# Pranav-Jain/Neural-Monte-Carlo-Fluid-Simulation

Hardware: AMD Instinct MI355X
Metric: WoS walk-steps/sec + pressure-projection wall-time per step, 2D karman 64k pts (higher is better)
Workload: dtype f32

## Files before the change

### include/wos.h

```cpp
#ifndef WOS_H
#define WOS_H

#include <stdint.h>

#ifdef __cplusplus
extern "C" {
#endif

#define WOS_ABI_VERSION 10

enum {
    WOS_OK = 0,
    WOS_E_INVALID = -1,
    WOS_E_IO = -2,
    WOS_E_DEVICE = -3,
    WOS_E_CAPACITY = -4,
    WOS_E_NOMEM = -5
};

#define WOS_PTRS_DEVICE 0x1u
#define WOS_ASYNC       0x2u

typedef struct wos_mesh {
    int32_t dim;
    int32_t n_vertices;
    int32_t n_prims;
    float *vertices;
    int32_t *prims;
} wos_mesh;

int wos_load_obj(const char *path, int32_t dim, int32_t flip_orientation,
                 int32_t normalize, wos_mesh *out);
void wos_mesh_free(wos_mesh *mesh);

typedef struct wos_scene_desc {
    int32_t dim;
    const float *vertices;
    const int32_t *prims;
    int32_t n_vertices, n_prims;
    const float *dvertices;
    const int32_t *dprims;
    int32_t n_dvertices, n_dprims;
    float dirichlet_value;
    float absorption;
    int32_t is_watertight;
    int32_t is_double_sided;
    const float *source;
    int32_t source_dims[3];
    int32_t source_on_device;
    const float *dirichlet_image;
    int32_t dirichlet_image_dims[2];
    float dirichlet_image_box[4];
    int32_t dirichlet_image_on_device;
    const float *neumann_image;
    int32_t neumann_image_dims[2];
    float neumann_image_box[4];
    int32_t neumann_image_on_device;
} wos_scene_desc;

typedef struct wos_scene wos_scene;

int wos_scene_create(const wos_scene_desc *desc, int32_t device, wos_scene **out);
int wos_scene_destroy(wos_scene *scene);

int wos_scene_set_source(wos_scene *scene, const float *source, const int32_t *dims,
                         int32_t on_device, void *stream);

#define WOS_MAX_CHANNELS 4
int wos_scene_set_source_channels(wos_scene *scene, const float *source, int32_t n_channels,
                                  const int32_t *dims, const float *dirichlet_values,
                                  int32_t on_device, void *stream);
int32_t wos_scene_channels(const wos_scene *scene);

int wos_release_caches(int32_t device);

int64_t wos_set_max_batch_tasks(int64_t max_tasks);

typedef struct wos_scene_info {
    int32_t dim, n_prims, n_silhouettes, n_dprims, device;
    float bbox_min[3], bbox_max[3];
} wos_scene_info;
int wos_scene_get_info(const wos_scene *scene, wos_scene_info *info);

enum { WOS_QUERY_NEUMANN = 0, WOS_QUERY_DIRICHLET = 1 };
int wos_scene_query(wos_scene *scene, int32_t which, float boundary_distance_mask,
                    const float *pts, int64_t n,
                    float *dist, float *signed_dist, float *closest , int32_t *state,
                    void *stream, uint32_t flags);

typedef struct wos_solver_params {
    int32_t n_walks;
    int32_t max_walk_length;
    int32_t steps_before_tikhonov;
    int32_t steps_before_maximal_spheres;
    float epsilon_shell;
    float min_star_radius;
    float silhouette_precision;
    float russian_roulette_threshold;
    float boundary_distance_mask;
    int32_t disable_gradient_control_variates;
    int32_t disable_gradient_antithetic_variates;
    int32_t use_cosine_sampling;
    int32_t ignore_dirichlet;
    int32_t ignore_neumann;
    int32_t ignore_source;
    uint64_t seed;
    int32_t robust_float;
    uint32_t schedule;
} wos_solver_params;

#define WOS_SCHED_GEOM_GLOBAL   0x1u
#define WOS_SCHED_FULL_NEUMANN  0x2u
#define WOS_SCHED_NO_STAR_GRID  0x4u
#define WOS_SCHED_NO_DIR_GRID   0x8u
#define WOS_SCHED_NO_TAIL_SPREAD 0x10u
#define WOS_SCHED_NO_GRID_SPREAD 0x20u

void wos_default_params(wos_solver_params *p);

typedef struct wos_stats {
    uint64_t walk_steps;
    uint64_t wasted_steps;
    uint64_t walks_recorded;
    uint64_t walks_escaped;
    uint64_t walks_max_length;
    uint64_t walks_rr;
    uint64_t walks_dirichlet;
    uint64_t points_estimated;
    uint64_t rejection_iters;
    double kernel_ms;
    double first_ball_ms;
    double walk_ms;
    double fold_ms;
    uint64_t walk_launches;
    int32_t first_ball_blocks_per_cu;
    int32_t walk_blocks_per_cu;
    int32_t walk_lds_bytes;
    int32_t star_grid;
    int32_t geom_global;
    int32_t dir_grid;
    uint64_t ticket;
} wos_stats;

int wos_solve(wos_scene *scene, const wos_solver_params *params,
              const float *pts, int64_t n, int64_t index_base, int64_t index_stride,
              float *p, float *grad, int32_t *n_est, int32_t *steps,
              wos_stats *stats, void *stream, uint32_t flags);

int wos_solve_var(wos_scene *scene, const wos_solver_params *params,
                  const float *pts, int64_t n, int64_t index_base, int64_t index_stride,
                  float *p, float *grad, float *p_var, float *grad_var, int32_t *n_est, int32_t *steps,
                  wos_stats *stats, void *stream, uint32_t flags);

int wos_solve_channels(wos_scene *scene, const wos_solver_params *params,
                       const float *pts, int64_t n, int64_t index_base, int64_t index_stride,
                       int32_t n_channels, float *p, float *grad, float *p_var, float *grad_var,
                       int32_t *n_est, int32_t *steps, wos_stats *stats, void *stream, uint32_t flags);

typedef struct wos_bvc_params {
    int32_t n_walks_solution;
// ... 102 lines not shown
```

### neural-monte-carlo-fluid-simulation_amd/csrc/wos_capi.hip

```cpp
#include <hip/hip_runtime.h>

#include <algorithm>
#include <cmath>
#include <list>
#include <cstdlib>
#include <cstring>
#include <memory>
#include <condition_variable>
#include <atomic>
#include <mutex>
#include <string>
#include <vector>

#include "../../include/wos.h"
#include "wos_bvc.h"
#include "wos_detmath.h"
#include "wos_host_scene.h"
#include "wos_launch.h"
#include "wos_siren.h"

namespace {

thread_local std::string g_err;

int fail(int code, const std::string& msg) {
  g_err = msg;
  return code;
}

#define HIP_TRY(expr)                                                                         \
  do {                                                                                        \
    hipError_t _e = (expr);                                                                   \
    if (_e != hipSuccess) return fail(WOS_E_DEVICE, std::string(#expr ": ") + hipGetErrorString(_e)); \
  } while (0)

template <typename T>
hipError_t upload(T** dst, const std::vector<T>& src) {
  *dst = nullptr;
  if (src.empty()) return hipSuccess;
  hipError_t e = hipMalloc((void**)dst, src.size() * sizeof(T));
  if (e != hipSuccess) { *dst = nullptr; return e; }
  e = hipMemcpy(*dst, src.data(), src.size() * sizeof(T), hipMemcpyHostToDevice);
  if (e != hipSuccess) {
    hipFree(*dst);
    *dst = nullptr;
  }
  return e;
}

struct StatSlot {
  uint64_t ticket = 0;
  unsigned long long* h_cnt = nullptr;
  hipEvent_t ev0 = nullptr, ev1 = nullptr, done = nullptr;
  std::vector<hipEvent_t> bev;
  int64_t n_batches = 0;
  int32_t bpc_fb = 0, bpc_walk = 0, walk_lds = 0, star_grid = 0, geom_global = 0, dir_grid = 0;
};
constexpr int kStatSlots = 16;

struct TaskWs {
  float* tasks = nullptr;
  int64_t task_cap = 0;
  int32_t* pstate = nullptr;
  int64_t pstate_cap = 0;
  unsigned long long* counters = nullptr;
  hipStream_t stream = nullptr;
  hipEvent_t done = nullptr;
};
constexpr int kSideWs = 2;

struct DevCtx {
  std::mutex mu;
  bool ready = false;
  int num_cus = 0;
  float* d_pts = nullptr;
  float* d_p = nullptr;
  float* d_g = nullptr;
  int32_t* d_nest = nullptr;
  int32_t* d_steps = nullptr;
  size_t ws_points = 0;
  float* d_pvar = nullptr;
  float* d_gvar = nullptr;
  size_t ws_var_points = 0;
  uint64_t* d_jump = nullptr;
  int n_jump = 0;
  float* d_tasks = nullptr;
  int64_t task_cap = 0;
  int32_t* d_pstate = nullptr;
  int64_t pstate_cap = 0;
  unsigned long long* d_counters = nullptr;
  StatSlot slot[kStatSlots];
  uint64_t next_ticket = 1;
  hipEvent_t done = nullptr;
  hipStream_t last_stream = nullptr;
  bool inflight = false;
  float* d_rejtab = nullptr;
  int stat_waiters = 0;
  std::condition_variable no_waiters;
  TaskWs side[kSideWs];
  hipStream_t bvc_dir = nullptr;
  hipEvent_t bvc_dir_done = nullptr;
};

constexpr int kMaxDevices = 64;
DevCtx g_ctx[kMaxDevices];

void ctx_free(DevCtx& c) {
  hipFree(c.d_pts); hipFree(c.d_p); hipFree(c.d_g); hipFree(c.d_nest); hipFree(c.d_steps);
  hipFree(c.d_pvar); hipFree(c.d_gvar);
  c.d_pvar = c.d_gvar = nullptr;
  c.ws_var_points = 0;
  hipFree(c.d_jump); hipFree(c.d_tasks); hipFree(c.d_pstate); hipFree(c.d_counters); hipFree(c.d_rejtab);
  c.d_rejtab = nullptr;
  for (StatSlot& q : c.slot) {
    if (q.ev0) hipEventDestroy(q.ev0);
    if (q.ev1) hipEventDestroy(q.ev1);
    if (q.done) hipEventDestroy(q.done);
    for (hipEvent_t e : q.bev) hipEventDestroy(e);
    if (q.h_cnt) hipHostFree(q.h_cnt);
    q = StatSlot{};
  }
  if (c.done) hipEventDestroy(c.done);
  if (c.bvc_dir_done) hipEventDestroy(c.bvc_dir_done);
  if (c.bvc_dir) hipStreamDestroy(c.bvc_dir);
  c.bvc_dir_done = nullptr;
  c.bvc_dir = nullptr;
  for (TaskWs& w : c.side) {
    hipFree(w.tasks); hipFree(w.pstate); hipFree(w.counters);
    if (w.done) hipEventDestroy(w.done);
    if (w.stream) hipStreamDestroy(w.stream);
    w = TaskWs{};
  }
  c.d_pts = c.d_p = c.d_g = nullptr;
  c.d_nest = c.d_steps = nullptr;
  c.ws_points = 0;
  c.d_jump = nullptr; c.n_jump = 0;
  c.d_tasks = nullptr; c.task_cap = 0;
  c.d_pstate = nullptr; c.pstate_cap = 0;
  c.d_counters = nullptr;
  c.done = nullptr;
  c.last_stream = nullptr;
  c.inflight = false;
  c.ready = false;
}

const std::vector<float>& rejection_tables() {
  static std::once_flag once;
  static std::vector<float> t(2 * wos::kRejTabBins);
  std::call_once(once, [] {
    wos::rejection_bound_table(2, t.data());
    wos::rejection_bound_table(3, t.data() + wos::kRejTabBins);
  });
  return t;
}

int ctx_ready(DevCtx& c, int device) {
  if (c.ready) return WOS_OK;
  {
    const std::vector<float>& t = rejection_tables();
    HIP_TRY(hipMalloc((void**)&c.d_rejtab, t.size() * sizeof(float)));
    HIP_TRY(hipMemcpy(c.d_rejtab, t.data(), t.size() * sizeof(float), hipMemcpyHostToDevice));
  }
  HIP_TRY(hipDeviceGetAttribute(&c.num_cus, hipDeviceAttributeMultiprocessorCount, device));
  HIP_TRY(hipMalloc((void**)&c.d_counters, wos::kMainCounterSlots * sizeof(unsigned long long)));
  for (StatSlot& q : c.slot) {
    HIP_TRY(hipHostMalloc((void**)&q.h_cnt, wos::kNumCounters * sizeof(unsigned long long)));
    HIP_TRY(hipEventCreate(&q.ev0));
    HIP_TRY(hipEventCreate(&q.ev1));
    HIP_TRY(hipEventCreateWithFlags(&q.done, hipEventDisableTiming));
  }
  HIP_TRY(hipEventCreateWithFlags(&c.done, hipEventDisableTiming));
  c.ready = true;
  return WOS_OK;
}

hipError_t ctx_order(DevCtx& c, hipStream_t st) {
  if (c.inflight && c.last_stream != st && c.done) return hipStreamWaitEvent(st, c.done, 0);
  return hipSuccess;
}

struct Geom {
  int device = 0;
  int dim = 2, double_sided = 0;
  std::vector<float> v, dv;
  std::vector<int32_t> ix, dix;
  wos::HostScene host;
  float *d_prim = nullptr, *d_paux = nullptr, *d_sil = nullptr, *d_dprim = nullptr, *d_dpaux = nullptr;
  float *d_pgroup = nullptr, *d_sgroup = nullptr, *d_dgroup = nullptr;
  float *d_ptree = nullptr, *d_stree = nullptr, *d_dtree = nullptr;
  float* d_nbox = nullptr;
  int32_t *d_nchild = nullptr, *d_nref = nullptr;
  std::mutex mu;
  struct Grid {
    float prec, min_r;
    bool ok;
    wos::StarGrid grid;
// ... 36 lines not shown
    std::lock_guard<std::mutex> lk(g_geom_mu);
    for (size_t i = 0; i < g_geom_lru.size(); i++)
      if (geom_matches(*g_geom_lru[i], d, device)) {
        out = g_geom_lru[i];
        std::rotate(g_geom_lru.begin(), g_geom_lru.begin() + i, g_geom_lru.begin() + i + 1);
        return WOS_OK;
      }
  }
  auto g = std::make_shared<Geom>();
  const int dim = d->dim;
  g->device = device;
  g->dim = dim;
  g->double_sided = d->is_double_sided;
  if (d->n_vertices > 0) g->v.assign(d->vertices, d->vertices + (size_t)d->n_vertices * dim);
  if (d->n_prims > 0) g->ix.assign(d->prims, d->prims + (size_t)d->n_prims * dim);
  if (d->n_dvertices > 0) g->dv.assign(d->dvertices, d->dvertices + (size_t)d->n_dvertices * dim);
  if (d->n_dprims > 0) g->dix.assign(d->dprims, d->dprims + (size_t)d->n_dprims * dim);
  wos::HostSceneInput in;
  in.dim = dim;
  in.vertices = d->vertices; in.prims = d->prims; in.n_vertices = d->n_vertices; in.n_prims = d->n_prims;
  in.dvertices = d->dvertices; in.dprims = d->dprims; in.n_dvertices = d->n_dvertices; in.n_dprims = d->n_dprims;
  in.is_double_sided = d->is_double_sided;
  std::string err;
  if (!wos::prepare_scene(in, g->host, err)) return fail(WOS_E_INVALID, "wos_scene_create: " + err);
  HIP_TRY(upload(&g->d_prim, g->host.prim));
  HIP_TRY(upload(&g->d_paux, g->host.paux));
  HIP_TRY(upload(&g->d_sil, g->host.sil));
  HIP_TRY(upload(&g->d_dprim, g->host.dprim));
  HIP_TRY(upload(&g->d_dpaux, g->host.dpaux));
  HIP_TRY(upload(&g->d_pgroup, g->host.pgroup));
  HIP_TRY(upload(&g->d_dgroup, g->host.dgroup));
  HIP_TRY(upload(&g->d_sgroup, g->host.sgroup));
  HIP_TRY(upload(&g->d_ptree, g->host.ptree.node));
  HIP_TRY(upload(&g->d_stree, g->host.stree.node));
  HIP_TRY(upload(&g->d_dtree, g->host.dtree.node));
  HIP_TRY(upload(&g->d_nbox, g->host.nbvh.box));
  HIP_TRY(upload(&g->d_nchild, g->host.nbvh.child));
  HIP_TRY(upload(&g->d_nref, g->host.nbvh.ref));
  {
    std::lock_guard<std::mutex> lk(g_geom_mu);
    g_geom_lru.insert(g_geom_lru.begin(), g);
    if (g_geom_lru.size() > kGeomCacheSize) g_geom_lru.pop_back();
  }
  out = g;
  return WOS_OK;
}

constexpr size_t kStarGridBudget = 16 * 1024;

constexpr size_t kLdsDynamicMax = 160 * 1024 - 4096;

int star_grid(Geom& g, float prec, float min_r, const Geom::Grid** out) {
  std::lock_guard<std::mutex> lk(g.mu);
  for (const Geom::Grid& x : g.grids)
    if (x.prec == prec && x.min_r == min_r) { *out = &x; return WOS_OK; }
  Geom::Grid x{prec, min_r, false, {}, nullptr};
  if (wos::build_star_grid(g.host, prec, min_r, kStarGridBudget, x.grid)) {
    HIP_TRY(upload(&x.d, x.grid.words));
    x.ok = true;
  }
  g.grids.push_back(std::move(x));
  *out = &g.grids.back();
  return WOS_OK;
}

int dir_grid(Geom& g, bool* ok) {
  std::lock_guard<std::mutex> lk(g.mu);
  if (!g.dgrid_built) {
    const bool have = wos::build_dirichlet_grid(g.host, g.dgrid);
    if (have) HIP_TRY(upload(&g.d_dgrid, g.dgrid.words));
    g.dgrid_ok = have;
    g.dgrid_built = true;
  }
  *ok = g.dgrid_ok;
  return WOS_OK;
}

#ifndef WOS_BATCH_LOG2
#define WOS_BATCH_LOG2 28
#endif
static_assert(WOS_BATCH_LOG2 <= 30, "task indices carry a flag in bit 31 (wos_walk_kernel hand-out)");
constexpr int64_t kDefaultBatchTasks = (int64_t)1 << WOS_BATCH_LOG2;
std::atomic<int64_t> g_max_batch_tasks{kDefaultBatchTasks};
std::atomic<uint64_t> g_scene_serial{0};

}

struct wos_scene {
  int device = 0;
  uint64_t serial = 0;
  std::shared_ptr<Geom> geom;
  wos::DevScene dev{};
  float* d_source = nullptr;
  size_t source_cap = 0;
  float* d_planar = nullptr;
  size_t planar_cap = 0;
  float g_dirichlet = 0.0f;
  float* d_dimg = nullptr;
  float* d_nimg = nullptr;
  std::mutex mu;
};

extern "C" {

const char* wos_last_error(void) { return g_err.c_str(); }
int32_t wos_abi_version(void) { return WOS_ABI_VERSION; }

int32_t wos_device_count(void) {
  int n = 0;
  if (hipGetDeviceCount(&n) != hipSuccess) return 0;
  return n;
}

int wos_load_obj(const char* path, int32_t dim, int32_t flip_orientation, int32_t normalize, wos_mesh* out) {
  if (!path || !out) return fail(WOS_E_INVALID, "wos_load_obj: null argument");
  if (dim != 2 && dim != 3) return fail(WOS_E_INVALID, "wos_load_obj: dim must be 2 or 3");
  std::vector<float> v;
  std::vector<int32_t> ix;
  std::string err;
  if (!wos::load_obj(path, dim, flip_orientation != 0, normalize != 0, v, ix, err))
    return fail(err.rfind("Error opening", 0) == 0 ? WOS_E_IO : WOS_E_INVALID, err);
  out->dim = dim;
  out->n_vertices = (int32_t)(v.size() / dim);
  out->n_prims = (int32_t)(ix.size() / dim);
  out->vertices = (float*)std::malloc(std::max<size_t>(1, v.size()) * sizeof(float));
  out->prims = (int32_t*)std::malloc(std::max<size_t>(1, ix.size()) * sizeof(int32_t));
  if (!out->vertices || !out->prims) return fail(WOS_E_NOMEM, "wos_load_obj: out of memory");
  if (!v.empty()) std::memcpy(out->vertices, v.data(), v.size() * sizeof(float));
  if (!ix.empty()) std::memcpy(out->prims, ix.data(), ix.size() * sizeof(int32_t));
  return WOS_OK;
}

void wos_mesh_free(wos_mesh* mesh) {
  if (!mesh) return;
  std::free(mesh->vertices);
  std::free(mesh->prims);
  mesh->vertices = nullptr;
  mesh->prims = nullptr;
  mesh->n_vertices = mesh->n_prims = 0;
}

void wos_default_params(wos_solver_params* p) {
  if (!p) return;
  std::memset(p, 0, sizeof(*p));
  p->n_walks = 128;
  p->max_walk_length = 1024;
  p->steps_before_tikhonov = 1024;
  p->steps_before_maximal_spheres = 1024;
  p->epsilon_shell = 1e-3f;
  p->min_star_radius = 1e-3f;
  p->silhouette_precision = 1e-3f;
  p->russian_roulette_threshold = 0.0f;
  p->boundary_distance_mask = 0.0f;
  p->seed = 0x5EED0001ULL;
}

static int check_source_dims(int dim, const int32_t* dims, size_t* nsrc) {
  const int nsd = dim == 2 ? 2 : 3;
  size_t n = 1;
  for (int k = 0; k < nsd; k++) {
    if (dims[k] <= 0) return fail(WOS_E_INVALID, "bad source dims");
    n *= (size_t)dims[k];
  }
  *nsrc = n;
  return WOS_OK;
}
// ... 162 lines not shown
  if (n_channels < 1 || n_channels > WOS_MAX_CHANNELS)
    return fail(WOS_E_INVALID, "wos_scene_set_source_channels: n_channels must be 1.." + std::to_string(WOS_MAX_CHANNELS) +
                                   ", got " + std::to_string(n_channels));
  if (dirichlet_values && s->d_dimg)
    return fail(WOS_E_INVALID, "wos_scene_set_source_channels: per-channel dirichlet_values cannot be combined with "
                               "the scene's Dirichlet image (image-valued data is shared by the channels)");
  if (n_channels == 1) {
    int rc = wos_scene_set_source(s, source, dims, on_device, stream);
    if (rc != WOS_OK) return rc;
    if (dirichlet_values) {
      std::lock_guard<std::mutex> lock(s->mu);
      s->dev.g_dirichlet = dirichlet_values[0];
      for (int c = 0; c < wos::kMaxChannels; c++) s->dev.g_ch[c] = dirichlet_values[0];
    }
    return WOS_OK;
  }
  size_t cells = 0;
  if (check_source_dims(s->dev.dim, dims, &cells) != WOS_OK)
    return fail(WOS_E_INVALID, "wos_scene_set_source_channels: bad source dims");
  std::lock_guard<std::mutex> lock(s->mu);
  HIP_TRY(hipSetDevice(s->device));
  hipStream_t st = (hipStream_t)stream;
  DevCtx& c = g_ctx[s->device];
  {
    std::lock_guard<std::mutex> lk(c.mu);
    HIP_TRY(ctx_order(c, st));
  }
  const size_t ntex = cells * wos::kMaxChannels, nplanar = cells * (size_t)n_channels;
  if (ntex > s->source_cap || (!on_device && nplanar > s->planar_cap)) HIP_TRY(hipStreamSynchronize(st));
  if (ntex > s->source_cap) {
    hipFree(s->d_source);
    s->d_source = nullptr;
    s->source_cap = 0;
    s->dev.source = nullptr;
    HIP_TRY(hipMalloc((void**)&s->d_source, ntex * sizeof(float)));
    s->source_cap = ntex;
  }
  const float* planar = source;
  if (!on_device) {
    if (nplanar > s->planar_cap) {
      hipFree(s->d_planar);
      s->d_planar = nullptr;
      s->planar_cap = 0;
      HIP_TRY(hipMalloc((void**)&s->d_planar, nplanar * sizeof(float)));
      s->planar_cap = nplanar;
    }
    HIP_TRY(hipMemcpyAsync(s->d_planar, source, nplanar * sizeof(float), hipMemcpyHostToDevice, st));
    planar = s->d_planar;
  }
  HIP_TRY(wos::launch_source_pack(planar, s->d_source, (int64_t)cells, n_channels, st));
  const int nsd = s->dev.dim == 2 ? 2 : 3;
  s->dev.source = s->d_source;
  for (int k = 0; k < 3; k++) s->dev.sdims[k] = k < nsd ? dims[k] : 1;
  s->dev.n_channels = n_channels;
  s->dev.g_dirichlet = s->g_dirichlet;
  for (int ch = 0; ch < wos::kMaxChannels; ch++)
    s->dev.g_ch[ch] = (dirichlet_values && ch < n_channels) ? dirichlet_values[ch] : s->g_dirichlet;
  return WOS_OK;
}

int32_t wos_scene_channels(const wos_scene* s) { return s ? s->dev.n_channels : 0; }

int wos_scene_destroy(wos_scene* s) {
  if (!s) return WOS_OK;
  {
    std::lock_guard<std::mutex> lock(s->mu);
    hipSetDevice(s->device);
    DevCtx& c = g_ctx[s->device];
    std::lock_guard<std::mutex> lk(c.mu);
    if (c.inflight) hipEventSynchronize(c.done);
    hipFree(s->d_source);
    hipFree(s->d_planar);
    hipFree(s->d_dimg);
    hipFree(s->d_nimg);
  }
  delete s;
  return WOS_OK;
}

int64_t wos_set_max_batch_tasks(int64_t max_tasks) {
  const int64_t v = max_tasks <= 0 ? kDefaultBatchTasks
                                   : std::min<int64_t>(std::max<int64_t>(max_tasks, (int64_t)1 << 16), (int64_t)1 << 30);
  return g_max_batch_tasks.exchange(v);
}

int wos_release_caches(int32_t device) {
  int ndev = 0;
  if (hipGetDeviceCount(&ndev) != hipSuccess) ndev = 0;
  for (int dv = 0; dv < std::min(ndev, kMaxDevices); dv++) {
    if (device >= 0 && dv != device) continue;
    DevCtx& c = g_ctx[dv];
    std::unique_lock<std::mutex> lk(c.mu);
    c.no_waiters.wait(lk, [&] { return c.stat_waiters == 0; });
    if (!c.ready) continue;
    HIP_TRY(hipSetDevice(dv));
    HIP_TRY(hipDeviceSynchronize());
    ctx_free(c);
  }
  std::lock_guard<std::mutex> lk(g_geom_mu);
  if (device < 0) {
    g_geom_lru.clear();
  } else {
    g_geom_lru.erase(std::remove_if(g_geom_lru.begin(), g_geom_lru.end(),
                                    [&](const std::shared_ptr<Geom>& g) { return g->device == device; }),
                     g_geom_lru.end());
  }
  return WOS_OK;
}

int wos_scene_get_info(const wos_scene* s, wos_scene_info* info) {
  if (!s || !info) return fail(WOS_E_INVALID, "wos_scene_get_info: null argument");
  const wos::HostScene& h = s->geom->host;
  info->dim = h.dim;
  info->n_prims = h.n_prims;
  info->n_silhouettes = h.n_sil;
  info->n_dprims = h.n_dprims;
  info->device = s->device;
  for (int k = 0; k < 3; k++) { info->bbox_min[k] = h.pmin[k]; info->bbox_max[k] = h.pmax[k]; }
  return WOS_OK;
}

int wos_scene_query(wos_scene* s, int32_t which, float boundary_distance_mask, const float* pts, int64_t n,
                    float* dist, float* signed_dist, float* closest, int32_t* state, void* stream, uint32_t flags) {
  if (!s) return fail(WOS_E_INVALID, "wos_scene_query: null scene");
  if (which != WOS_QUERY_NEUMANN && which != WOS_QUERY_DIRICHLET)
    return fail(WOS_E_INVALID, "wos_scene_query: which must be WOS_QUERY_NEUMANN (0) or WOS_QUERY_DIRICHLET (1), got " +
                                   std::to_string(which));
  if (!dist && !signed_dist && !closest && !state)
    return fail(WOS_E_INVALID, "wos_scene_query: no output requested (dist, signed_dist, closest and state are all null)");
  if (n < 0) return fail(WOS_E_INVALID, "wos_scene_query: negative point count");
  if (n >= (int64_t)0xFFFFFFF0LL) return fail(WOS_E_INVALID, "wos_scene_query: too many points for one call");
  const wos::HostScene& host = s->geom->host;
  const int dim = host.dim;
  if ((dist || signed_dist || closest) && (which == WOS_QUERY_NEUMANN ? host.n_prims : host.n_dprims) <= 0)
    return fail(WOS_E_INVALID, std::string("wos_scene_query: the scene holds no ") +
                                   (which == WOS_QUERY_NEUMANN ? "Neumann" : "Dirichlet") +
                                   " boundary (dist, signed_dist and closest need one; state alone does not)");
  if (n == 0) return WOS_OK;
  if (!pts) return fail(WOS_E_INVALID, "wos_scene_query: null point buffer");
  wos::DevScene dsc;
  {
    std::lock_guard<std::mutex> lock(s->mu);
    dsc = s->dev;
  }
  HIP_TRY(hipSetDevice(s->device));
  hipStream_t st = (hipStream_t)stream;
  if (flags & WOS_PTRS_DEVICE) {
    HIP_TRY(wos::launch_point_query(dim, dsc, which, boundary_distance_mask, pts, n, dist, signed_dist, closest,
                                    state, st));
    if (!(flags & WOS_ASYNC)) HIP_TRY(hipStreamSynchronize(st));
    return WOS_OK;
  }
  const size_t N = (size_t)n;
  const size_t o_dist = N * dim, o_sd = o_dist + (dist ? N : 0), o_cl = o_sd + (signed_dist ? N : 0),
               o_st = o_cl + (closest ? N * dim : 0), total = o_st + (state ? N : 0);
  float* tmp = nullptr;
  if (hipMalloc((void**)&tmp, total * sizeof(float)) != hipSuccess)
    return fail(WOS_E_NOMEM, "wos_scene_query: cannot allocate " + std::to_string(total * sizeof(float)) +
                                 " bytes of staging");
  const auto run = [&]() -> hipError_t {
    hipError_t e = hipMemcpyAsync(tmp, pts, N * dim * sizeof(float), hipMemcpyHostToDevice, st);
    if (e != hipSuccess) return e;
    e = wos::launch_point_query(dim, dsc, which, boundary_distance_mask, tmp, n, dist ? tmp + o_dist : nullptr,
                                signed_dist ? tmp + o_sd : nullptr, closest ? tmp + o_cl : nullptr,
                                state ? (int32_t*)(tmp + o_st) : nullptr, st);
    if (e != hipSuccess) return e;
// ... 193 lines not shown
      dsc.sgrid = gr->d;
      dsc.sgrid_words = (int32_t)gr->grid.words.size();
      dsc.sgrid_off_words = gr->grid.off_words;
      for (int k = 0; k < 3; k++) {
        dsc.sgrid_n[k] = gr->grid.n[k];
        dsc.sgrid_min[k] = gr->grid.gmin[k];
        dsc.sgrid_inv[k] = gr->grid.inv[k];
      }
    }
  }
  dsc.dgrid = nullptr;
  if (!(prm->schedule & WOS_SCHED_NO_DIR_GRID) && host.dim == 2 && host.n_dprims > 0) {
    bool ok = false;
    int rc = dir_grid(geom, &ok);
    if (rc != WOS_OK) return rc;
    if (ok) {
      dsc.dgrid = geom.d_dgrid;
      dsc.dgrid_off_words = geom.dgrid.off_words;
      for (int k = 0; k < 2; k++) {
        dsc.dgrid_n[k] = geom.dgrid.n[k];
        dsc.dgrid_min[k] = geom.dgrid.gmin[k];
        dsc.dgrid_inv[k] = geom.dgrid.inv[k];
      }
    }
  }
  const int dir_floats = ((host.n_dprims * PS + 3) & ~3) + wos::kGroupStride * host.n_dgroups;
  L.geom_floats_walk = L.geom_floats + ((dsc.sgrid_words + 3) & ~3) + dir_floats;
  L.shmem_walk = (size_t)L.geom_floats_walk * sizeof(float) + wos::kWavesPerBlockHost * wos::walk_wave_lds_bytes(dim);
  if (dsc.sgrid != nullptr && L.shmem_walk > kLdsDynamicMax) {
    dsc.sgrid = nullptr;
    dsc.sgrid_words = dsc.sgrid_off_words = 0;
    L.geom_floats_walk = L.geom_floats + dir_floats;
    L.shmem_walk =
        (size_t)L.geom_floats_walk * sizeof(float) + wos::kWavesPerBlockHost * wos::walk_wave_lds_bytes(dim);
  }
  return WOS_OK;
}

struct DevBufs {
  std::vector<void*> p;
  ~DevBufs() { for (void* q : p) hipFree(q); }
  template <typename T>
  hipError_t get(T** out, size_t n) {
    *out = nullptr;
    void* q = nullptr;
    hipError_t e = hipMalloc(&q, std::max<size_t>(1, n) * sizeof(T));
    if (e == hipSuccess) { p.push_back(q); *out = (T*)q; }
    return e;
  }
};

wos::DevParams dev_params(const wos_solver_params* prm) {
  wos::DevParams dp{};
  const bool anti = !prm->disable_gradient_antithetic_variates;
  dp.n_walks = prm->n_walks;
  dp.n_anti = anti ? 2 : 1;
  dp.n_pairs = anti ? std::max(1, prm->n_walks / 2) : prm->n_walks;
  dp.max_walk_length = prm->max_walk_length;
  dp.steps_before_tikhonov = prm->steps_before_tikhonov;
  dp.steps_before_maximal_spheres = prm->steps_before_maximal_spheres;
  dp.epsilon_shell = prm->epsilon_shell;
  dp.min_star_radius = prm->min_star_radius;
  dp.silhouette_precision = prm->silhouette_precision;
  dp.rr_threshold = prm->russian_roulette_threshold;
  dp.boundary_distance_mask = prm->boundary_distance_mask;
  dp.use_cv = !prm->disable_gradient_control_variates;
  dp.use_cosine = prm->use_cosine_sampling;
  dp.ignore_dirichlet = prm->ignore_dirichlet;
  dp.ignore_neumann = prm->ignore_neumann;
  dp.ignore_source = prm->ignore_source;
  dp.robust = prm->robust_float != 0;
  dp.seed = prm->seed;
  return dp;
}

struct SolveExtra {
  const float* ddir = nullptr;
  float* deriv = nullptr;
  bool force_estimate = false;
  int wave_prio = 0;
  float* p_var = nullptr;
  float* grad_var = nullptr;
  int channels = 1;
};

int solve_locked(wos_scene* s, const wos_solver_params* prm, const float* pts, int64_t n, int64_t index_base,
                 int64_t index_stride, float* p, float* grad, int32_t* n_est, int32_t* steps, wos_stats* stats,
                 void* stream, uint32_t flags, const SolveExtra& ex);
int solve_checked(wos_scene* s, const wos_solver_params* prm, const float* pts, int64_t n, int64_t index_base,
                  int64_t index_stride, int32_t n_channels, float* p, float* grad, float* p_var, float* grad_var,
                  int32_t* n_est, int32_t* steps, wos_stats* stats, void* stream, uint32_t flags);

}

extern "C" {

int wos_solve_var(wos_scene* s, const wos_solver_params* prm, const float* pts, int64_t n, int64_t index_base,
                  int64_t index_stride, float* p, float* grad, float* p_var, float* grad_var, int32_t* n_est,
                  int32_t* steps, wos_stats* stats, void* stream, uint32_t flags) {
  return solve_checked(s, prm, pts, n, index_base, index_stride, 0, p, grad, p_var, grad_var, n_est, steps, stats,
                       stream, flags);
}

int wos_solve_channels(wos_scene* s, const wos_solver_params* prm, const float* pts, int64_t n, int64_t index_base,
                       int64_t index_stride, int32_t n_channels, float* p, float* grad, float* p_var,
                       float* grad_var, int32_t* n_est, int32_t* steps, wos_stats* stats, void* stream,
                       uint32_t flags) {
  if (n_channels < 1 || n_channels > WOS_MAX_CHANNELS)
    return fail(WOS_E_INVALID, "wos_solve_channels: n_channels must be 1.." + std::to_string(WOS_MAX_CHANNELS) +
                                   ", got " + std::to_string(n_channels));
  return solve_checked(s, prm, pts, n, index_base, index_stride, n_channels, p, grad, p_var, grad_var, n_est, steps,
                       stats, stream, flags);
}

}

namespace {

int solve_checked(wos_scene* s, const wos_solver_params* prm, const float* pts, int64_t n, int64_t index_base,
                  int64_t index_stride, int32_t n_channels, float* p, float* grad, float* p_var, float* grad_var,
                  int32_t* n_est, int32_t* steps, wos_stats* stats, void* stream, uint32_t flags) {
  if (!s || !prm) return fail(WOS_E_INVALID, "wos_solve: null scene/params");
  if (n < 0) return fail(WOS_E_INVALID, "wos_solve: negative point count");
  if (n > 0 && (!pts || !p || !grad)) return fail(WOS_E_INVALID, "wos_solve: null point/output buffer");
  if (n >= (int64_t)0xFFFFFFF0LL) return fail(WOS_E_INVALID, "wos_solve: too many points for one call");
  if (prm->n_walks < 1) return fail(WOS_E_INVALID, "wos_solve: nWalks must be >= 1");
  if (prm->max_walk_length < 0) return fail(WOS_E_INVALID, "wos_solve: maxWalkLength must be >= 0");
  if (!(prm->epsilon_shell >= 0.0f) || !(prm->min_star_radius >= 0.0f) || !(prm->silhouette_precision >= 0.0f))
    return fail(WOS_E_INVALID, "wos_solve: negative tolerance");
  std::lock_guard<std::mutex> lock(s->mu);
  HIP_TRY(hipSetDevice(s->device));
  DevCtx& c = g_ctx[s->device];
  std::lock_guard<std::mutex> lk(c.mu);
  if (n_channels == 0 && s->dev.n_channels > 1)
    return fail(WOS_E_INVALID, "wos_solve: the scene holds " + std::to_string(s->dev.n_channels) +
                                   " source channels; use wos_solve_channels (or wos_scene_set_source for one)");
  if (n_channels != 0 && n_channels != s->dev.n_channels)
    return fail(WOS_E_INVALID, "wos_solve_channels: n_channels " + std::to_string(n_channels) +
                                   " differs from the scene's " + std::to_string(s->dev.n_channels));
  SolveExtra ex;
  ex.p_var = p_var;
  ex.grad_var = grad_var;
  ex.channels = s->dev.n_channels;
  return solve_locked(s, prm, pts, n, index_base, index_stride, p, grad, n_est, steps, stats, stream, flags, ex);
}

}

extern "C" {

int wos_solve(wos_scene* s, const wos_solver_params* prm, const float* pts, int64_t n, int64_t index_base,
              int64_t index_stride, float* p, float* grad, int32_t* n_est, int32_t* steps, wos_stats* stats,
              void* stream, uint32_t flags) {
  return wos_solve_var(s, prm, pts, n, index_base, index_stride, p, grad, nullptr, nullptr, n_est, steps, stats,
                       stream, flags);
}

}

namespace {

#ifndef WOS_LHS_JUMP_STAGE
#define WOS_LHS_JUMP_STAGE 1
#endif
struct SolvePlan {
  wos::DevParams dp{};
// ... 22 lines not shown
    dp.rej_tab = c.d_rejtab;
  }

  WalkLayout wl;
  {
    int rc = walk_layout(s, prm, wl);
    if (rc != WOS_OK) return rc;
  }
  wos::DevScene& dsc = P.dsc;
  dsc = wl.dsc;
  P.geom_floats_walk = wl.geom_floats_walk;
  P.shmem_walk = wl.shmem_walk;
  P.lhs_floats = ((2 * dp.n_pairs * (dim - 1)) + 3) & ~3;
  P.shmem_fb = wos::kWavesPerBlockHost * wos::first_ball_wave_lds_bytes(P.lhs_floats, dp.n_pairs);
  P.shmem_fb_run = P.shmem_fb;
  wos::DevScene& dfb = P.dfb;
  dfb = s->dev;
  dfb.dgrid = dsc.dgrid;
  dfb.dgrid_off_words = dsc.dgrid_off_words;
  for (int k = 0; k < 2; k++) {
    dfb.dgrid_n[k] = dsc.dgrid_n[k];
    dfb.dgrid_min[k] = dsc.dgrid_min[k];
    dfb.dgrid_inv[k] = dsc.dgrid_inv[k];
  }
  if ((prm->schedule & WOS_SCHED_GEOM_GLOBAL) || P.shmem_walk > kLdsDynamicMax) {
    dfb.geom_global = 1;
    dsc.geom_global = 1;
    P.geom_floats_walk = 0;
    P.shmem_walk = wos::kWavesPerBlockHost * wos::walk_wave_lds_bytes(dim);
  }
  if (P.shmem_fb > kLdsDynamicMax)
    return fail(WOS_E_CAPACITY, "wos_solve: nWalks exceed the LDS budget of the first-ball kernel (" +
                                    std::to_string(P.shmem_fb) + " bytes of stratified samples per block)");
  if (P.shmem_walk > kLdsDynamicMax)
    return fail(WOS_E_CAPACITY, "wos_solve: the walk kernel's per-wave scratch exceeds the LDS budget (" +
                                    std::to_string(P.shmem_walk) + " bytes)");

  P.wpp = (int64_t)dp.n_pairs * dp.n_anti;
  {
    double diag2 = 0.0;
    for (int k = 0; k < 3; k++) diag2 += (double)host.ext[k] * host.ext[k];
    const double mu_r = std::sqrt(std::max(0.0, (double)s->dev.absorption)) * std::sqrt(diag2) * 1.01;
    dp.neumann_inert = (!dp.robust && s->dev.watertight && !s->dev.double_sided && mu_r < 80.0 && !s->dev.nimg &&
                        !(prm->schedule & WOS_SCHED_FULL_NEUMANN)) ? 1 : 0;
  }
  dp.tail_spread = (dim == 2 && !dp.robust && !dsc.geom_global && !(prm->schedule & WOS_SCHED_NO_TAIL_SPREAD)) ? 1 : 0;
#ifdef WOS_ACCT_NOSPREAD
  dp.tail_spread = 0;
#endif
  if (record) {
    dp.neumann_inert = 0;
    dp.tail_spread = 0;
    dsc.n_channels = 1;
    dfb.n_channels = 1;
  }
  P.kv = wos::kernel_variant(dim, dsc, dp, false);
  return WOS_OK;
}

int solve_grids(DevCtx& c, int dim, int64_t chunk, bool record, SolvePlan& P) {
  wos::DevParams& dp = P.dp;
  const bool gg = P.dsc.geom_global != 0;
  const auto occupancy = [&](int which, size_t shmem, int* blocks) {
    return record ? wos::occupancy_rec_blocks_per_cu(dim, gg, which, shmem, blocks)
                  : wos::occupancy_blocks_per_cu(P.kv, which, shmem, blocks);
  };
  HIP_TRY(occupancy(0, P.shmem_fb, &P.bpc_fb));
  const int jn = std::min(2 * (2 * dp.n_pairs) * (dim - 1), wos::kLhsJumpMax);
  const size_t shmem_j = P.shmem_fb + (size_t)jn * 2 * sizeof(uint64_t);
  int bpc_j = 0;
  if (jn > 0 && shmem_j <= kLdsDynamicMax) HIP_TRY(occupancy(0, shmem_j, &bpc_j));
  if (WOS_LHS_JUMP_STAGE && jn > 0 && bpc_j >= P.bpc_fb) {
    dp.lhs_jump_n = jn;
    P.shmem_fb_run = shmem_j;
  }
  const int64_t fb_waves = (chunk + wos::first_ball_points_per_wave(dp.n_pairs) - 1) / wos::first_ball_points_per_wave(dp.n_pairs);
  P.grid_fb = (int)std::min<int64_t>((fb_waves + wos::kWavesPerBlockHost - 1) / wos::kWavesPerBlockHost,
                                     (int64_t)std::max(1, P.bpc_fb) * std::max(1, c.num_cus));
  HIP_TRY(occupancy(1, P.shmem_walk, &P.bpc_walk));
  P.grid_walk = std::max(1, P.bpc_walk) * std::max(1, c.num_cus);
  return WOS_OK;
}

int solve_locked(wos_scene* s, const wos_solver_params* prm, const float* pts, int64_t n, int64_t index_base,
                 int64_t index_stride, float* p, float* grad, int32_t* n_est, int32_t* steps, wos_stats* stats,
                 void* stream, uint32_t flags, const SolveExtra& ex) {
  Geom& geom = *s->geom;
  const wos::HostScene& host = geom.host;
  const int dim = host.dim;
  hipStream_t st = (hipStream_t)stream;
  DevCtx& c = g_ctx[s->device];
  {
    int rc = ctx_ready(c, s->device);
    if (rc != WOS_OK) return rc;
  }

  SolvePlan plan;
  {
    int rc = solve_plan(c, s, prm, ex, false, plan);
    if (rc != WOS_OK) return rc;
  }
  wos::DevParams& dp = plan.dp;
  const wos::DevScene& dsc = plan.dsc;
  const wos::DevScene& dfb = plan.dfb;
  const int geom_floats_walk = plan.geom_floats_walk, lhs_floats = plan.lhs_floats;
  const size_t shmem_walk = plan.shmem_walk;
  const wos::KernelVariant kv = plan.kv;

  HIP_TRY(ctx_order(c, st));

  const float* d_pts = pts;
  float* d_p = p;
  float* d_g = grad;
  int32_t* d_nest = n_est;
  int32_t* d_steps = steps;
  float* d_pvar = ex.p_var;
  float* d_gvar = ex.grad_var;
  const bool dev_ptrs = (flags & WOS_PTRS_DEVICE) != 0;
  const int C = ex.channels;
  if (!dev_ptrs && n > 0) {
    int rc = ensure_workspace(c, dim, (size_t)n * C);
    if (rc != WOS_OK) return rc;
    HIP_TRY(hipMemcpyAsync(c.d_pts, pts, (size_t)n * dim * sizeof(float), hipMemcpyHostToDevice, st));
    d_pts = c.d_pts; d_p = c.d_p; d_g = c.d_g;
    d_nest = n_est ? c.d_nest : nullptr;
    d_steps = steps ? c.d_steps : nullptr;
    if (ex.p_var || ex.grad_var) {
      rc = ensure_var_workspace(c, (size_t)n * C);
      if (rc != WOS_OK) return rc;
      d_pvar = ex.p_var ? c.d_pvar : nullptr;
      d_gvar = ex.grad_var ? c.d_gvar : nullptr;
    }
  }

  const int64_t wpp = (int64_t)dp.n_pairs * dp.n_anti;
  const int64_t chunk = std::max<int64_t>(1, std::min<int64_t>(n, g_max_batch_tasks.load() / wpp));
  const int64_t n_chunks = n > 0 ? (n + chunk - 1) / chunk : 0;
  if (n > 0) {
    int rc = ensure_tasks(c, dim, chunk * wpp, chunk, C);
    if (rc != WOS_OK) return rc;
    rc = solve_grids(c, dim, chunk, false, plan);
    if (rc != WOS_OK) return rc;
  }
  const int grid_fb = plan.grid_fb, grid_walk = plan.grid_walk, bpc_fb = plan.bpc_fb, bpc_walk = plan.bpc_walk;
  const size_t shmem_fb_run = plan.shmem_fb_run;
  const uint64_t ticket = c.next_ticket++;
  StatSlot& q = c.slot[ticket % kStatSlots];
  while ((int64_t)q.bev.size() < 4 * n_chunks) {
    hipEvent_t e = nullptr;
    HIP_TRY(hipEventCreate(&e));
    q.bev.push_back(e);
  }
  q.ticket = ticket;
  q.n_batches = n_chunks;
  q.bpc_fb = bpc_fb;
  q.bpc_walk = bpc_walk;
  q.walk_lds = (int32_t)shmem_walk;
  q.star_grid = dsc.sgrid != nullptr;
  q.geom_global = dsc.geom_global;
  q.dir_grid = dsc.dgrid != nullptr;
  HIP_TRY(hipEventRecord(q.ev0, st));
  if (n_chunks == 0) HIP_TRY(wos::launch_zero(c.d_counters, wos::kMainCounterSlots, nullptr, 0, st));
  for (int64_t k = 0; k < n_chunks; k++) {
    const int64_t b0 = k * chunk;
    hipEvent_t* ev = &q.bev[4 * k];
    const int64_t nb = std::min(chunk, n - b0);
    wos::DevTasks tk = task_view(c, dim, nb * wpp, (int32_t)wpp, C);
    tk.ddir = ex.ddir ? ex.ddir + b0 * dim : nullptr;
    tk.deriv = ex.deriv ? ex.deriv + b0 : nullptr;
    const int64_t bbase = index_base + b0 * index_stride;
    unsigned long long* qslot = c.d_counters + wos::kNumCounters;
    unsigned int* q_points = (unsigned int*)qslot;
    unsigned int* q_tasks = (unsigned int*)(c.d_counters + wos::kTaskQueueSlot0);
    const int walk_grid = (int)std::min<int64_t>(grid_walk, (tk.T + 63) / 64);
    HIP_TRY(wos::launch_zero(k == 0 ? c.d_counters : qslot,
                             k == 0 ? wos::kNumCounterSlots : wos::kNumCounterSlots - wos::kNumCounters,
                             tk.hist, 2 * wos::kCostBuckets, st));
    HIP_TRY(hipEventRecord(ev[0], st));
    HIP_TRY(wos::launch_point_setup(dim, dfb, dp, d_pts + b0 * dim, nb, tk, st));
    HIP_TRY(wos::launch_lpt_order(tk, nb, st));
    HIP_TRY(wos::launch_first_balls(kv, dfb, dp, d_pts + b0 * dim, nb, bbase, index_stride, tk, c.d_counters,
                                    q_points, grid_fb, shmem_fb_run, lhs_floats, st));
    HIP_TRY(hipEventRecord(ev[1], st));
    HIP_TRY(wos::launch_walks(kv, dsc, dp, tk, bbase, index_stride, c.d_counters, q_tasks, walk_grid,
                              shmem_walk, geom_floats_walk, st));
    HIP_TRY(hipEventRecord(ev[2], st));
    for (int ch = 0; ch < C; ch++) {
      wos::DevTasks tkc = tk;
      tkc.total = tk.total + (int64_t)ch * tk.T;
      tkc.first = tk.first + (int64_t)ch * tk.T;
      const int64_t o1 = (int64_t)ch * n + b0, od = ((int64_t)ch * n + b0) * dim;
      HIP_TRY(wos::launch_fold(dim, dp, tkc, nb, d_p + o1, d_g + od, (d_nest && ch == 0) ? d_nest + b0 : nullptr,
                               (d_steps && ch == 0) ? d_steps + b0 : nullptr, d_pvar ? d_pvar + o1 : nullptr,
                               d_gvar ? d_gvar + od : nullptr, st));
    }
    HIP_TRY(hipEventRecord(ev[3], st));
  }
  HIP_TRY(hipEventRecord(q.ev1, st));
  HIP_TRY(hipMemcpyAsync(q.h_cnt, c.d_counters, wos::kNumCounters * sizeof(unsigned long long),
                         hipMemcpyDeviceToHost, st));
  if (!dev_ptrs && n > 0) {
    HIP_TRY(hipMemcpyAsync(p, d_p, (size_t)n * C * sizeof(float), hipMemcpyDeviceToHost, st));
    HIP_TRY(hipMemcpyAsync(grad, d_g, (size_t)n * C * dim * sizeof(float), hipMemcpyDeviceToHost, st));
    if (n_est) HIP_TRY(hipMemcpyAsync(n_est, d_nest, (size_t)n * sizeof(int32_t), hipMemcpyDeviceToHost, st));
    if (steps) HIP_TRY(hipMemcpyAsync(steps, d_steps, (size_t)n * sizeof(int32_t), hipMemcpyDeviceToHost, st));
    if (ex.p_var)
      HIP_TRY(hipMemcpyAsync(ex.p_var, d_pvar, (size_t)n * C * sizeof(float), hipMemcpyDeviceToHost, st));
    if (ex.grad_var)
      HIP_TRY(hipMemcpyAsync(ex.grad_var, d_gvar, (size_t)n * C * dim * sizeof(float), hipMemcpyDeviceToHost, st));
  }
  HIP_TRY(hipEventRecord(q.done, st));
  HIP_TRY(hipEventRecord(c.done, st));
  c.last_stream = st;
  c.inflight = true;
  if ((flags & WOS_ASYNC) && dev_ptrs) {
    if (stats) {
      *stats = wos_stats{};
      stats->ticket = ticket;
    }
    return WOS_OK;
  }
  HIP_TRY(hipStreamSynchronize(st));
  c.inflight = false;
  wos::diag_dump(dim == 2 ? "2d" : "3d");
  if (stats) {
    int rc = fill_stats(q, stats);
    if (rc != WOS_OK) return rc;
  }
  return WOS_OK;
}

}

extern "C" {

int wos_solve_stats(wos_scene* s, uint64_t ticket, wos_stats* stats) {
  if (!s || !stats) return fail(WOS_E_INVALID, "wos_solve_stats: null scene/stats");
  const auto unknown = [&] {
    return fail(WOS_E_INVALID, "wos_solve_stats: unknown ticket (more than " + std::to_string(kStatSlots) +
                                   " solves were enqueued on this device after it)");
  };
  HIP_TRY(hipSetDevice(s->device));
  DevCtx& c = g_ctx[s->device];
  hipEvent_t done = nullptr;
  {
    std::lock_guard<std::mutex> lock(s->mu);
    std::lock_guard<std::mutex> lk(c.mu);
    StatSlot& q = c.slot[ticket % kStatSlots];
    if (ticket == 0 || q.ticket != ticket) return unknown();
    done = q.done;
    c.stat_waiters++;
  }
  const hipError_t e = hipEventSynchronize(done);
  std::lock_guard<std::mutex> lock(s->mu);
  std::lock_guard<std::mutex> lk(c.mu);
  if (--c.stat_waiters == 0) c.no_waiters.notify_all();
  if (e != hipSuccess) return fail(WOS_E_DEVICE, std::string("wos_solve_stats: ") + hipGetErrorString(e));
  StatSlot& q = c.slot[ticket % kStatSlots];
  if (q.ticket != ticket) return unknown();
  HIP_TRY(hipEventSynchronize(q.done));
  return fill_stats(q, stats);
}

}

// ... 888 lines not shown

  std::vector<float> recs;
  recs.reserve((size_t)(nb + nd_keep) * wos::kBvcRec);
  for (int64_t i = 0; i < nb; i++) {
    const bool al = smp.aligned[i] != 0, dir = smp.dirichlet[i] != 0;
    const int kind = dir ? (al ? wos::kBvcDirichletAligned : wos::kBvcDirichlet) : (al ? wos::kBvcAligned : wos::kBvcBoundary);
    const float r[wos::kBvcRec] = {smp.bpt[2 * i], smp.bpt[2 * i + 1], smp.bnrm[2 * i], smp.bnrm[2 * i + 1],
                                   al ? smp.pdf_aligned : smp.pdf_main, 0.0f, 0.0f, (float)kind};
    recs.insert(recs.end(), r, r + wos::kBvcRec);
  }
  for (int64_t i = 0; i < nd; i++) {
    if (!dkeep[i]) continue;
    const float r[wos::kBvcRec] = {smp.dcand[2 * i], smp.dcand[2 * i + 1], 0.0f, 0.0f, smp.pdf_domain, dsrc[i], 0.0f,
                                   (float)wos::kBvcDomain};
    recs.insert(recs.end(), r, r + wos::kBvcRec);
  }
  const int64_t nd_kept = nd_keep;
  const int64_t nrec = nb + nd_kept;
  float *d_recs = nullptr, *d_state = nullptr;
  HIP_TRY(B.get(&d_recs, (size_t)nrec * wos::kBvcRec));
  HIP_TRY(B.get(&d_state, (size_t)18 * ne));
  if (nrec > 0) HIP_TRY(hipMemcpy(d_recs, recs.data(), recs.size() * sizeof(float), hipMemcpyHostToDevice));

  WalkLayout wl;
  wos_solver_params wp0 = *prm;
  {
    int rc = walk_layout(s, &wp0, wl);
    if (rc != WOS_OK) return rc;
  }
  wos::DevScene dsc = wl.dsc;
  if ((prm->schedule & WOS_SCHED_GEOM_GLOBAL) || wl.shmem_walk > kLdsDynamicMax) {
    dsc.geom_global = 1;
    wl.geom_floats_walk = 0;
    wl.shmem_walk = wos::kWavesPerBlockHost * wos::walk_wave_lds_bytes(2);
  }
  const bool dir_solve = has_dir && !bp->use_finite_differences;
  wos_solver_params gp = *prm;
  gp.n_walks = bp->n_walks_gradient;
  gp.boundary_distance_mask = 0.0f;
  {
    int rc = ensure_jump(c, std::max(4096, 4 * std::max(1, bp->n_walks_gradient)));
    if (rc != WOS_OK) return rc;
  }
  int64_t side_tasks[kSideWs] = {0, 0}, side_points[kSideWs] = {0, 0};
  const int64_t max_batch = g_max_batch_tasks.load();
  for (const Run& r : runs) {
    const int64_t m = r.b1 - r.b0;
    if (!r.dir || bp->use_finite_differences) {
      const int64_t w = r.dir ? bp->n_walks_gradient : bp->n_walks_solution;
      if (m * w > max_batch) return fail(WOS_E_CAPACITY, "wos_bvc: samples x nWalks exceed one task batch");
      side_tasks[0] = std::max(side_tasks[0], m * w);
      side_points[0] = std::max(side_points[0], m);
    } else if (dir_solve) {
      const int64_t wpp = gp.disable_gradient_antithetic_variates ? gp.n_walks : 2 * std::max(1, gp.n_walks / 2);
      const int64_t chunk = std::max<int64_t>(1, std::min<int64_t>(m, max_batch / wpp));
      int rc = ensure_tasks(c, 2, chunk * wpp, chunk);
      if (rc != WOS_OK) return rc;
    }
  }
  if (nn * bp->n_walks_solution > max_batch)
    return fail(WOS_E_CAPACITY, "wos_bvc: samples x nWalks exceed one task batch");
  side_tasks[1] = nn * bp->n_walks_solution;
  side_points[1] = nn;
  for (int k = 0; k < kSideWs; k++) {
    TaskWs& w = c.side[k];
    int rc = side_ready(w, bvc_priority(k == 0));
    if (rc == WOS_OK) rc = ensure_tasks_in(w.tasks, w.task_cap, w.pstate, w.pstate_cap, 2, side_tasks[k], side_points[k]);
    if (rc != WOS_OK) return rc;
  }
  if (!c.bvc_dir) HIP_TRY(hipStreamCreateWithPriority(&c.bvc_dir, hipStreamNonBlocking, bvc_priority(true)));
  if (!c.bvc_dir_done) HIP_TRY(hipEventCreateWithFlags(&c.bvc_dir_done, hipEventDisableTiming));
  HIP_TRY(hipEventRecord(q.bev[1], st));
  HIP_TRY(hipStreamWaitEvent(c.bvc_dir, q.bev[1], 0));
  for (TaskWs& w : c.side) {
    HIP_TRY(hipStreamWaitEvent(w.stream, q.bev[1], 0));
    HIP_TRY(wos::launch_zero(w.counters, wos::kNumCounterSlots, nullptr, 0, w.stream));
  }

  std::vector<uint64_t> dtickets;
  if (dir_solve) {
    SolveExtra ex;
    ex.force_estimate = true;
    ex.wave_prio = 2;
    for (const Run& r : runs) {
      if (!r.dir) continue;
      ex.ddir = d_ddir + 2 * r.b0;
      ex.deriv = d_bdn + r.b0;
      wos_stats rs{};
      int rc = solve_locked(s, &gp, d_bpt + 2 * r.b0, r.b1 - r.b0, r.b0, 1, d_bsol + r.b0, d_dgrad, d_bnest + r.b0,
                            nullptr, &rs, c.bvc_dir, WOS_PTRS_DEVICE | WOS_ASYNC, ex);
      if (rc != WOS_OK) return rc;
      dtickets.push_back(rs.ticket);
    }
  }
  HIP_TRY(hipEventRecord(c.bvc_dir_done, c.bvc_dir));

  bool first_walk[kSideWs] = {true, true};
  auto walks = [&](int k, const float* pts_d, const float* nrm_d, const uint8_t* al_d, const float* dd_d, int64_t np_,
                   int64_t base, int n_walks, int on_neumann, uint32_t tag, float* sol_d, int32_t* nest_d) -> int {
    if (np_ <= 0) return WOS_OK;
    TaskWs& w = c.side[k];
    wos_solver_params wp = *prm;
    wp.n_walks = n_walks;
    wp.disable_gradient_antithetic_variates = 1;
    wos::DevParams dp = dev_params(&wp);
    dp.jump = c.d_jump;
    dp.n_jump = c.n_jump;
    dp.rej_tab = c.d_rejtab;
    dp.wave_prio = k == 0 ? 3 : 0;
    const int64_t wpp = n_walks;
    wos::DevTasks tk = task_view_in(w.tasks, w.pstate, w.pstate_cap, 2, np_ * wpp, (int32_t)wpp);
    tk.n0 = tk.bdir;
    tk.r0 = tk.first;
    tk.sflags = reinterpret_cast<uint32_t*>(tk.sdir);
    if (!first_walk[k])
      HIP_TRY(wos::launch_zero(w.counters + wos::kNumCounters, wos::kNumCounterSlots - wos::kNumCounters, nullptr, 0,
                               w.stream));
    first_walk[k] = false;
    HIP_TRY(wos::launch_bvc_start(dsc, dp, pts_d, nrm_d, al_d, dd_d, np_, tk, on_neumann, tag, w.stream));
    int bpc = 0;
    const wos::KernelVariant kv = wos::kernel_variant(2, dsc, dp, true);
    HIP_TRY(wos::occupancy_blocks_per_cu(kv, 1, wl.shmem_walk, &bpc));
    const int grid = (int)std::min<int64_t>((int64_t)std::max(1, bpc) * std::max(1, c.num_cus), (tk.T + 63) / 64);
    unsigned int* q_tasks = (unsigned int*)(w.counters + wos::kTaskQueueSlot0);
    HIP_TRY(wos::launch_walks(kv, dsc, dp, tk, base, 1, w.counters, q_tasks, grid, wl.shmem_walk,
                              wl.geom_floats_walk, w.stream));
    HIP_TRY(wos::launch_bvc_fold(tk, np_, sol_d, nest_d, w.stream));
    q.bpc_walk = bpc;
    return WOS_OK;
  };
  for (const Run& r : runs) {
    const int64_t m = r.b1 - r.b0;
    int rc = WOS_OK;
    if (!r.dir)
      rc = walks(0, d_bpt + 2 * r.b0, d_bnrm + 2 * r.b0, d_al + r.b0, d_bdd + r.b0, m, r.b0, bp->n_walks_solution, 1,
                 6u, d_bsol + r.b0, d_bnest + r.b0);
    else if (bp->use_finite_differences)
      rc = walks(0, d_bpt + 2 * r.b0, d_bnrm + 2 * r.b0, d_al + r.b0, d_bdd + r.b0, m, r.b0, bp->n_walks_gradient, 0,
                 8u, d_bsol + r.b0, d_bnest + r.b0);
    if (rc != WOS_OK) return rc;
    if (r.dir && bp->use_finite_differences)
      HIP_TRY(wos::launch_bvc_fd(s->dev, d_bpt + 2 * r.b0, d_bsol + r.b0, m, d_bdn + r.b0, c.side[0].stream));
  }
  {
    int rc = walks(1, d_npt, nullptr, nullptr, d_ndd, nn, 0, bp->n_walks_solution, 0, 7u, d_nsol, d_nnest);
    if (rc != WOS_OK) return rc;
  }
  q.walk_lds = (int32_t)wl.shmem_walk;
  q.star_grid = dsc.sgrid != nullptr;
  q.geom_global = dsc.geom_global;
  q.dir_grid = dsc.dgrid != nullptr;

  int64_t p1 = nb;
  if (dir_solve)
    for (int64_t i = 0; i < nb; i++)
      if (smp.dirichlet[i]) { p1 = i; break; }
  const float ab = s->dev.absorption;
  const bool part1 = p1 > 0, part1_last = p1 == nrec;
  if (part1) {
    HIP_TRY(wos::launch_bvc_fill(d_recs, 0, p1, d_bsol, d_bdn, s->dev, prm->ignore_neumann, c.side[0].stream));
    HIP_TRY(wos::launch_bvc_splat(d_recs, 0, (int)p1, 1, part1_last ? 1 : 0, d_state, d_slist, d_scount, d_ept, ne,
                                  ab, bp->radius_clamp, bp->kernel_regularization, d_sol, d_grad, c.side[0].stream));
  }
  for (TaskWs& w : c.side) HIP_TRY(hipEventRecord(w.done, w.stream));
  HIP_TRY(hipStreamWaitEvent(st, c.bvc_dir_done, 0));
  HIP_TRY(hipStreamWaitEvent(st, c.side[0].done, 0));
// ... 345 lines not shown
```

### neural-monte-carlo-fluid-simulation_amd/csrc/wos_device.h

```cpp

#pragma once
#include <cstdio>

#include "wos_detmath.h"
#include "wos_scene.h"

namespace wos {

#ifndef WOS_DIAG
#define WOS_DIAG 0
#endif

constexpr int kWave = 64;
constexpr int kBlock = 256;

enum { WC_DIRICHLET = 0, WC_RR = 1, WC_MAXLEN = 2, WC_ESCAPED = 3 };

enum { C_STEPS = 0, C_WASTED, C_REC, C_ESC, C_MAXL, C_RR, C_DIR, C_PTS, C_ITERS, C_NUM };

__device__ __forceinline__ void wave_sync() {
  __builtin_amdgcn_fence(__ATOMIC_SEQ_CST, "wavefront");
  __builtin_amdgcn_wave_barrier();
}

// ... 3108 lines not shown
  const bool maskG = (!inside && !sc.double_sided) || __builtin_fabsf(nDist) < mask;
  const float bd = smin(dDist, nDist);
  int bucket = 0;
  if (estimate) {
    const float l2 = __builtin_amdgcn_logf(smax(bd, 1e-9f));
    bucket = (int)sclamp((int)(-2.0f * l2) + 8, 1, kCostBuckets - 1);
  }
  *bucket_out = bucket;
  *firstR = 0.99f * bd;
  return (estimate ? kPtEstimate : 0) | (maskP ? kPtMaskP : 0) | (maskG ? kPtMaskG : 0) | (bucket << 8);
}

#ifndef WOS_SETUP_LANES
#define WOS_SETUP_LANES 1
#endif
constexpr int kSetupLanes = WOS_SETUP_LANES;
#ifndef WOS_SETUP_LDS_FLOATS
#define WOS_SETUP_LDS_FLOATS 4096
#endif
constexpr int kSetupLdsFloats = WOS_SETUP_LDS_FLOATS;
static_assert((kSetupLanes & (kSetupLanes - 1)) == 0 && kSetupLanes <= kWave, "kSetupLanes");
template <int DIM>
__global__ __launch_bounds__(256) void wos_point_setup_kernel(const DevScene sc, const DevParams prm,
                                                             const float* __restrict__ pts, int64_t n,
                                                             const DevTasks tk) {
  __shared__ uint32_t s_hist[kCostBuckets];
  __shared__ __attribute__((aligned(16))) float s_prim[kSetupLdsFloats];
  constexpr int PS = Layout<DIM>::prim;
  const int nfl = sc.n_prims * PS, dfl = sc.n_dprims * PS;
  const bool lds_n = nfl <= kSetupLdsFloats, lds_d = nfl + dfl <= kSetupLdsFloats;
  if (lds_n)
    for (int k = threadIdx.x; k < nfl; k += blockDim.x) s_prim[k] = sc.prim[k];
  if (lds_d)
    for (int k = threadIdx.x; k < dfl; k += blockDim.x) s_prim[nfl + k] = sc.dprim[k];
  if (threadIdx.x < kCostBuckets) s_hist[threadIdx.x] = 0u;
  __syncthreads();
  const float* nprim = lds_n ? s_prim : sc.prim;
  const float* dprim = lds_d ? s_prim + nfl : sc.dprim;
  const int64_t gi = (int64_t)blockIdx.x * blockDim.x + threadIdx.x;
  const int64_t i = gi / kSetupLanes;
  const int sub = (int)(gi % kSetupLanes);
  if (i < n) {
    float x[DIM];
    for (int k = 0; k < DIM; k++) x[k] = pts[i * DIM + k];
    float nDist = kFltMax, nSigned = kFltMax;
    if (sc.n_prims > 0) {
      const Closest c = closest_lane<DIM>(nprim, sc.pgroup, sc.n_prims, sc.n_pgroups, x, sub, kSetupLanes);
      nDist = c.d;
      nSigned = signed_dist<DIM>(sc.paux, c, x);
    }
    float dDist, dSigned;
    if (sc.n_dprims > 0) {
      const Closest c = closest_lane<DIM>(dprim, sc.dgroup, sc.n_dprims, sc.n_dgroups, x, sub, kSetupLanes);
      dDist = c.d;
      dSigned = signed_dist<DIM>(sc.dpaux, c, x);
    } else {
      dDist = dSigned = bbox_far_dist<DIM>(sc, x);
    }
    int bucket;
    float firstR;
    const int32_t ps = point_state<DIM>(sc, prm, nDist, nSigned, dDist, dSigned, &bucket, &firstR);
    if (sub == 0) {
      tk.pstate[i] = ps;
      tk.prad[i] = firstR;
      if constexpr (DIM == 2) {
        if (tk.pball != nullptr && !prm.robust && (ps & kPtEstimate) && sc.absorption > 0.0f &&
            prm.steps_before_tikhonov == 0) {
          Gfn<2> g;
          g.init(true, sc.absorption);
          g.update_ball(x, firstR, false);
          tk.pball[i] = g.A0;
          tk.pball[tk.pball_stride + i] = g.A1;
          tk.pball[2 * tk.pball_stride + i] = g.B0;
          tk.pball[3 * tk.pball_stride + i] = g.B1;
        }
      }
      atomicAdd(&s_hist[bucket], 1u);
    }
  }
  __syncthreads();
  if (threadIdx.x < kCostBuckets && s_hist[threadIdx.x]) atomicAdd(&tk.hist[threadIdx.x], s_hist[threadIdx.x]);
}

template <int DIM, bool RB = false, int NC = 1>
__global__ __launch_bounds__(kBlock) __attribute__((amdgpu_waves_per_eu(DIM == 2 ? WOS_FB_WAVES_PER_EU2 : WOS_FB_WAVES_PER_EU))) void wos_first_ball_kernel(
    const DevScene sc, const DevParams prm, const float* __restrict__ pts, int64_t n, int64_t base, int64_t stride,
    const DevTasks tk, unsigned long long* __restrict__ counters, unsigned int* __restrict__ work, int lhs_floats) {
  constexpr bool REC = false;
  const DevTape* const tape = nullptr;
#include "wos_first_ball_body.inc"
}

__device__ __forceinline__ void wave_priority(int level) {
  if (level == 1) __builtin_amdgcn_s_setprio(1);
  else if (level == 2) __builtin_amdgcn_s_setprio(2);
  else if (level >= 3) __builtin_amdgcn_s_setprio(3);
}

template <int DIM, bool BSTART, bool RB, int NC, bool REC>
__device__ __forceinline__ void walk_start(const DevScene& sc, const DevParams& prm, const DevTasks& tk, int64_t t,
                                           uint32_t pidx, uint32_t w, const float* v_pt, float v_thr, const float* v_tsrc,
                                           float v_dd, int64_t base, int64_t stride, bool yuk0, WalkState<DIM, NC, REC>& st,
                                           Gfn<DIM, RB>& g, Pcg32& ws, float& ddist, uint32_t& wsteps, float& firstR) {
  for (int kk = 0; kk < DIM; kk++) { st.pt[kk] = v_pt[kk]; st.n[kk] = 0.0f; st.prevDir[kk] = 0.0f; }
  st.prevDist = 0.0f;
  st.throughput = v_thr;
  st.onNeumann = false;
  st.walkLength = 0;
  st.totalNeumann = 0.0f;
  for (int c = 0; c < NC; c++) st.totalSource[c] = v_tsrc[c];
  st.pend = false;
  if constexpr (REC) {
    st.rbase = st.tape->slot[t];
    st.rcap = st.tape->slot[t + 1] - st.rbase;
    st.rn = 0u;
  }
  ddist = v_dd;
  g.init(yuk0, sc.absorption);
  if constexpr (BSTART) {
    for (int kk = 0; kk < DIM; kk++) { st.n[kk] = tk.n0[kk * tk.T + t]; st.prevDir[kk] = st.n[kk]; }
    st.prevDist = kFltMax;
    const uint32_t fl = tk.sflags[t];
    st.onNeumann = (fl & 1u) != 0u;
    firstR = tk.r0[t];
    ws.seed(seed32(prm.seed, (uint64_t)(base + (int64_t)pidx * stride), (uint64_t)w, (fl >> 8) & 0xFFu));
    wsteps = 0;
  } else {
    ws.seed(seed32(prm.seed, (uint64_t)(base + (int64_t)pidx * stride), (uint64_t)w, 2));
    wsteps = 1;
  }
}

template <int DIM, bool GG, bool BSTART, bool RB, bool NEU = true, int NC, bool REC>
__device__ __forceinline__ int walk_iteration(const DevScene& sc, const DevParams& prm, const LGeom& G, bool active,
                                              WalkState<DIM, NC, REC>& st, Gfn<DIM, RB>& gc, Pcg32& ws, float& ddist,
                                              uint32_t& wsteps, float& firstR, StarLDS<DIM>* starL,
                                              RayLDS<DIM>* rayL, RejLDS* rejL, uint32_t* c_iters, int lane) {
  DIAG_T0(t_step);
  Gfn<DIM, RB> g;
  g.yukawa = gc.yukawa; g.lambda = sc.absorption; g.sqrtLambda = __builtin_sqrtf(sc.absorption);
  int code = -1;
  DIAG_LONE(lone, active);
  bool flip = false, query = false;
  if (active) code = walk_step_begin<DIM>(sc, prm, ddist, st, &flip, &query, BSTART ? firstR : 0.0f);
  DIAG_T0(t_star);
  const float starQ = star_radius_wave<DIM, GG>(G, sc, prm, active && code < 0 && query, st.pt, ddist, flip, starL, lane);
  if (WOS_PROBE & 8) {
    float px[DIM];
    for (int k = 0; k < DIM; k++) px[k] = probe_opaque(st.pt[k]);
    probe_sink(star_radius_wave<DIM, GG>(G, sc, prm, active && code < 0 && query, px, probe_opaque(ddist), flip, starL,
                                         lane));
  }
  DIAG_ADD_LONE(D_STAR, D_L_STAR, t_star, lone);
  const bool live = active && code < 0;
  float dir[DIM], org[DIM], starR = 0.0f;
  for (int k = 0; k < DIM; k++) { dir[k] = 1.0f; org[k] = 0.0f; }
  DIAG_T0(t_mid);
  if (live) starR = walk_step_mid<DIM>(prm, ddist, ws, g, st, &wsteps, query, starQ, dir, org, BSTART ? firstR : 0.0f);
  DIAG_ADD_LONE(D_MID, D_L_MID, t_mid, lone);
  Hit ip;
  DIAG_T0(t_ray);
  const bool hit = ray_hit_wave<DIM, GG>(G, sc, live, org, dir, starR, &ip, rayL, lane);
  if (WOS_PROBE & 16) {
    Hit ip2;
    float po[DIM];
    for (int k = 0; k < DIM; k++) po[k] = probe_opaque(org[k]);
    probe_sink(ray_hit_wave<DIM, GG>(G, sc, live, po, dir, probe_opaque(starR), &ip2, rayL, lane) ? ip2.d : 0.0f);
  }
  DIAG_ADD_LONE(D_RAY, D_L_RAY, t_ray, lone);
  DIAG_T0(t_end);
// ... 386 lines not shown
```

### neural-monte-carlo-fluid-simulation_amd/csrc/wos_first_ball_body.inc

```
  extern __shared__ __attribute__((aligned(16))) float smem[];
  const int lane = threadIdx.x & (kWave - 1);
  const int wave = threadIdx.x / kWave;
  const int npairs = prm.n_pairs;
  const int P = fb_points_per_wave(npairs);
  const int wave_floats = 2 * P * lhs_floats + (int)(fb_union_bytes(P * lhs_floats, 2 * npairs) / sizeof(float));
  float* wbase = smem + wave * wave_floats;
  unsigned long long* ljump = reinterpret_cast<unsigned long long*>(smem + (int)(blockDim.x / kWave) * wave_floats);
  stage_rej_jump(prm);
  for (int i = threadIdx.x; i < 2 * prm.lhs_jump_n; i += blockDim.x) ljump[i] = prm.jump[i];
#if WOS_DIAG
  if (threadIdx.x < D_NUM) s_diag[threadIdx.x] = 0u;
#endif
  __syncthreads();
  RejLDS* rejL = reinterpret_cast<RejLDS*>(wbase + 2 * P * lhs_floats);
  const int span = P > 1 ? npairs : kWave;
  const int slot = P > 1 ? lane / npairs : 0;
  const int wl = lane - slot * span;
  const bool used = slot < P;
  const int myslot = used ? slot : 0;

  uint32_t c_iters = 0, c_pts = 0;
  const bool yuk0 = sc.absorption > 0.0f && prm.steps_before_tikhonov == 0;

  const unsigned int take = kPtGrab * (unsigned int)P;
  unsigned int idx = 0;
  if (lane == 0) idx = atomicAdd(work, take);
  idx = __shfl(idx, 0);
  unsigned int cend = idx + take;
  float xn[DIM], rn = 0.0f;
  bool en = false;
  const bool pre = !RB && DIM == 2 && yuk0;
  float bn[4] = {0.0f, 0.0f, 0.0f, 0.0f};
  {
    const unsigned int li = idx + (unsigned int)myslot;
    for (int k = 0; k < DIM; k++) xn[k] = (int64_t)li < n ? pts[(int64_t)li * DIM + k] : 0.0f;
    if ((int64_t)li < n) {
      rn = tk.prad[li];
      en = (tk.pstate[li] & kPtEstimate) != 0;
      if (pre)
        for (int k = 0; k < 4; k++) bn[k] = tk.pball[k * tk.pball_stride + li];
    }
  }
  for (;;) {
    if ((int64_t)idx >= n) break;
    float x[DIM];
    for (int k = 0; k < DIM; k++) x[k] = xn[k];
    float firstR = rn;
    const bool estimate = en && used;
    float pb[4];
    for (int k = 0; k < 4; k++) pb[k] = bn[k];
    const bool grab = idx + (unsigned int)P >= cend;
    unsigned int nidx_l0 = 0;
    if (grab && lane == 0) nidx_l0 = atomicAdd(work, take);
    DIAG_T0(t_fb0);
    unsigned int nidx, ncend = cend;
    if (grab) {
      nidx = (unsigned int)__shfl((int)nidx_l0, 0);
      ncend = nidx + take;
    } else {
      nidx = idx + (unsigned int)P;
    }
    {
      const unsigned int li = nidx + (unsigned int)myslot;
      for (int k = 0; k < DIM; k++) xn[k] = (int64_t)li < n ? pts[(int64_t)li * DIM + k] : 0.0f;
      en = false;
      if ((int64_t)li < n) {
        rn = tk.prad[li];
        en = (tk.pstate[li] & kPtEstimate) != 0;
        if (pre)
          for (int k = 0; k < 4; k++) bn[k] = tk.pball[k * tk.pball_stride + li];
      }
    }
    const uint64_t em = __ballot(estimate && wl == 0);
    if (em == 0) { idx = nidx; cend = ncend; continue; }
    c_pts += lane == 0 ? (uint32_t)__popcll(em) : 0u;
    DIAG_ADD(D_FB_SETUP, t_fb0);
    DIAG_COUNT(D_FB_PTS, __popcll(em));
    DIAG_T0(t_fb1);
    const bool all = lhs_all_fits(npairs, DIM, P);
    for (int s = 0; s < P; s++) {
      if (!all && !((em >> (s * span)) & 1ull)) continue;
      float* strat_s = wbase + 2 * s * lhs_floats;
      build_lhs<DIM>(prm, ljump, base + (int64_t)(idx + (unsigned int)s) * stride, strat_s,
                     reinterpret_cast<int*>(strat_s + lhs_floats), reinterpret_cast<char*>(rejL), lane, !all);
    }
    if constexpr (DIM == 3)
      if (all) {
        const int ns = 2 * npairs;
        const int* part0 = reinterpret_cast<const int*>(wbase + lhs_floats);
        if (ns <= kWave) lhs_permute_reg<DIM - 1, 1, 4>(wbase, part0, 2 * lhs_floats, 0, P * (DIM - 1), ns, lane);
        else lhs_permute_reg<DIM - 1, 2, 2>(wbase, part0, 2 * lhs_floats, 0, P * (DIM - 1), ns, lane);
      }
    DIAG_ADD(D_FB_LHS, t_fb1);
    DIAG_T0(t_fb2);
    const int fs = (int)(__builtin_ctzll(em) / (unsigned)span);
    const int es = estimate ? myslot : fs;
    if (!estimate) {
      for (int k = 0; k < DIM; k++) x[k] = lane_bcast(x[k], fs * span);
      firstR = lane_bcast(firstR, fs * span);
      for (int k = 0; k < 4; k++) pb[k] = lane_bcast(pb[k], fs * span);
    }
    const unsigned int pidx = idx + (unsigned int)es;
    const int64_t gidx = base + (int64_t)pidx * stride;
    const float* strat = wbase + 2 * es * lhs_floats;
    const int wend = P > 1 ? 1 : npairs;
    for (int w0 = 0; w0 < wend; w0 += kWave) {
      const int w = w0 + wl;
      first_balls<DIM, RB, NC, REC>(sc, prm, tk, x, firstR, strat, gidx, estimate && w < npairs, w,
                                    (int64_t)pidx * tk.wpp + (int64_t)w * prm.n_anti, yuk0, &c_iters, rejL, lane,
                                    pb, tk.ddir ? tk.ddir + (int64_t)pidx * DIM : nullptr, tape);
    }
    DIAG_ADD(D_FB_BALLS, t_fb2);
    DIAG_ADD(D_FB_TOTAL, t_fb0);
    DIAG_MAX(D_FB_MAX, __builtin_amdgcn_s_memtime() - t_fb0);
    wave_sync();
    idx = nidx;
    cend = ncend;
  }
  flush_counter(counters, C_ITERS, c_iters, lane);
  flush_counter(counters, C_PTS, c_pts, lane);
#if WOS_DIAG
  __syncthreads();
  if (threadIdx.x < D_NUM) {
    if (diag_is_max(threadIdx.x)) atomicMax(&g_diag[threadIdx.x], s_diag[threadIdx.x]);
    else atomicAdd(&g_diag[threadIdx.x], s_diag[threadIdx.x]);
  }
#endif
```

### neural-monte-carlo-fluid-simulation_amd/csrc/wos_kernel.hip

```cpp
#include "wos_device.h"
#include <algorithm>
#include "wos_launch.h"
#include "wos_select.h"

namespace wos {

__global__ __launch_bounds__(256) void wos_lpt_scatter_kernel(const DevTasks tk, int64_t n) {
  __shared__ uint32_t cnt[kCostBuckets], base[kCostBuckets], off[kCostBuckets];
  if (threadIdx.x < kCostBuckets) {
    cnt[threadIdx.x] = 0u;
    uint32_t acc = 0;
    for (int b = kCostBuckets - 1; b > (int)threadIdx.x; b--) acc += tk.hist[b];
    off[threadIdx.x] = acc;
  }
  __syncthreads();
  const int64_t i = (int64_t)blockIdx.x * blockDim.x + threadIdx.x;
  int b = 0;
  uint32_t local = 0;
  if (i < n) {
    b = (tk.pstate[i] >> 8) & (kCostBuckets - 1);
    local = atomicAdd(&cnt[b], 1u);
  }
  __syncthreads();
  if (threadIdx.x < kCostBuckets && cnt[threadIdx.x])
// ... 10 lines not shown
  X(2, true, false, false, false, false, 1)   \
  X(2, false, false, false, true, true, 1)    \
  X(2, false, false, false, false, true, 1)   \
  X(3, false, false, false, true, false, 1)   \
  X(3, false, false, false, false, false, 1)  \
  X(3, true, false, false, true, false, 1)    \
  X(3, true, false, false, false, false, 1)
UNIT_FIRST_BALLS(WOS_FIRST_BALL_INSTANTIATE)
template __global__ void wos_point_setup_kernel<2>(const DevScene, const DevParams, const float*, int64_t,
                                                   const DevTasks);
template __global__ void wos_point_setup_kernel<3>(const DevScene, const DevParams, const float*, int64_t,
                                                   const DevTasks);
UNIT_WALKS(WOS_WALK_INSTANTIATE)
UnitKernels unit_kernels_plain(const KernelVariant& v) {
  UnitKernels k;
  UNIT_FIRST_BALLS(WOS_FIRST_BALL_SELECT)
  UNIT_WALKS(WOS_WALK_SELECT)
  return k;
}
template __global__ void wos_fold_kernel<2>(const DevParams, const DevTasks, int64_t, float*, float*, int32_t*,
                                            int32_t*);
template __global__ void wos_fold_kernel<3>(const DevParams, const DevTasks, int64_t, float*, float*, int32_t*,
                                            int32_t*);
template __global__ void wos_fold4_kernel<3>(const DevParams, const DevTasks, int64_t, float*, float*, int32_t*,
                                             int32_t*, float*, float*);
template __global__ void wos_fold4_kernel<2>(const DevParams, const DevTasks, int64_t, float*, float*, int32_t*,
                                             int32_t*, float*, float*);
template __global__ void wos_fold4_kernel<3, true>(const DevParams, const DevTasks, int64_t, float*, float*,
                                                   int32_t*, int32_t*, float*, float*);
template __global__ void wos_fold4_kernel<2, true>(const DevParams, const DevTasks, int64_t, float*, float*,
                                                   int32_t*, int32_t*, float*, float*);

__global__ void wos_math_selftest_kernel(int which, const double* x, double* out, int64_t n) {
  int64_t i = (int64_t)blockIdx.x * blockDim.x + threadIdx.x;
  if (i >= n) return;
  double v = x[i], r = 0.0;
  switch (which) {
    case 0: r = dexp(v); break;
    case 1: r = dlog(v); break;
    case 2: { double s, c; dsincos(v, &s, &c); r = s; } break;
    case 3: { double s, c; dsincos(v, &s, &c); r = c; } break;
    case 4: r = datan(v); break;
    case 5: r = __builtin_sqrt(v); break;
    case 6: r = bessi0(v); break;
    case 7: r = bessi1(v); break;
    case 8: r = bessk0(v); break;
    case 9: r = bessk1(v); break;
    case 10: r = (double)fexp((float)v); break;
    case 11: r = (double)flog((float)v); break;
    case 12: r = (double)fsin((float)v); break;
    case 13: r = (double)fcos((float)v); break;
    case 14: r = (double)fcbrt((float)v); break;
    case 15: r = (double)__builtin_sqrtf((float)v); break;
    case 16: r = (double)i0_fast((float)v); break;
    case 17: r = (double)k0_fast((float)v); break;
    case 18: { double a, b; bessel_ik<true, false>(v, &r, &a, nullptr, nullptr); (void)b; } break;
    case 19: { double a; bessel_ik<false, true>(v, nullptr, nullptr, &r, &a); } break;
    case 20: { double a; bessel_ik<true, false>(v, &a, &r, nullptr, nullptr); } break;
    case 21: { double a; bessel_ik<false, true>(v, nullptr, nullptr, &a, &r); } break;
    case 22: { double a, b, c; bessel_ik<true, true>(v, &a, &r, &b, &c); } break;
    case 23: { double a, b, c; bessel_ik<true, true>(v, &a, &b, &c, &r); } break;
    case 24: { float k, i; k0i0_fast((float)v, &k, &i); r = (double)i; } break;
    case 25: { float k, i; k0i0_fast((float)v, &k, &i); r = (double)k; } break;
    default: r = __builtin_nan("");
  }
  out[i] = r;
}


static UnitKernels kernels_of(const KernelVariant& v) {
  UnitKernels k;
  for (UnitKernels (*unit)(const KernelVariant&) : {unit_kernels_plain, unit_kernels_channels, unit_kernels_robust,
                                                    unit_kernels_channels_rb, unit_kernels_bstart}) {
    const UnitKernels u = unit(v);
    if (u.first_ball) k.first_ball = u.first_ball;
    if (u.walk) k.walk = u.walk;
  }
  return k;
}

hipError_t launch_first_balls(const KernelVariant& v, const DevScene& sc, const DevParams& prm, const float* pts,
                              int64_t n, int64_t base, int64_t stride, const DevTasks& tk,
                              unsigned long long* counters, unsigned int* work, int grid, size_t shmem, int lhs_floats,
                              hipStream_t s) {
  const FirstBallKernel kernel = kernels_of(v).first_ball;
  if (!kernel) return hipErrorInvalidValue;
  hipLaunchKernelGGL(kernel, dim3(grid), dim3(kBlock), shmem, s, sc, prm, pts, n, base, stride, tk, counters, work,
                     lhs_floats);
  return hipGetLastError();
}

hipError_t launch_point_setup(int dim, const DevScene& sc, const DevParams& prm, const float* pts, int64_t n,
                              const DevTasks& tk, hipStream_t s) {
  const int grid = (int)((n * kSetupLanes + 255) / 256);
  if (grid < 1) return hipSuccess;
  if (dim == 2) hipLaunchKernelGGL(wos_point_setup_kernel<2>, dim3(grid), dim3(256), 0, s, sc, prm, pts, n, tk);
  else hipLaunchKernelGGL(wos_point_setup_kernel<3>, dim3(grid), dim3(256), 0, s, sc, prm, pts, n, tk);
  return hipGetLastError();
}

__global__ __launch_bounds__(256) void wos_zero_kernel(unsigned long long* a, int n64, uint32_t* b, int n32) {
  const int i0 = blockIdx.x * blockDim.x + threadIdx.x, di = gridDim.x * blockDim.x;
  for (int i = i0; i < n64; i += di) a[i] = 0ull;
  for (int i = i0; i < n32; i += di) b[i] = 0u;
}

hipError_t launch_zero(unsigned long long* a, int n64, uint32_t* b, int n32, hipStream_t s) {
  const int grid = std::max(1, std::min(32, (std::max(n64, n32 / 2) + 1023) / 1024));
  hipLaunchKernelGGL(wos_zero_kernel, dim3(grid), dim3(256), 0, s, a, n64, b, n32);
  return hipGetLastError();
}

hipError_t launch_lpt_order(const DevTasks& tk, int64_t n, hipStream_t s) {
  const int grid = (int)((n + 255) / 256);
  if (grid > 0) hipLaunchKernelGGL(wos_lpt_scatter_kernel, dim3(grid), dim3(256), 0, s, tk, n);
  return hipGetLastError();
}

hipError_t launch_walks(const KernelVariant& v, const DevScene& sc, const DevParams& prm, const DevTasks& tk,
                        int64_t base, int64_t stride, unsigned long long* counters, unsigned int* tqueue, int grid,
                        size_t shmem, int geom_floats, hipStream_t s) {
  const WalkKernel kernel = kernels_of(v).walk;
  if (!kernel) return hipErrorInvalidValue;
  hipLaunchKernelGGL(kernel, dim3(grid), dim3(kBlock), shmem, s, sc, prm, tk, base, stride, counters, tqueue,
                     geom_floats);
  return hipGetLastError();
}

hipError_t launch_fold(int dim, const DevParams& prm, const DevTasks& tk, int64_t n, float* p, float* g,
                       int32_t* nest, int32_t* steps, float* p_var, float* g_var, hipStream_t s) {
  if (tk.deriv == nullptr) {
    const int g4 = (int)((n + kFold4Points - 1) / kFold4Points);
    if (g4 < 1) return hipSuccess;
    const dim3 blk(4 * kFold4Points);
    if (p_var || g_var) {
      if (dim == 3)
        hipLaunchKernelGGL((wos_fold4_kernel<3, true>), dim3(g4), blk, 0, s, prm, tk, n, p, g, nest, steps, p_var, g_var);
      else
        hipLaunchKernelGGL((wos_fold4_kernel<2, true>), dim3(g4), blk, 0, s, prm, tk, n, p, g, nest, steps, p_var, g_var);
    } else if (dim == 3) {
      hipLaunchKernelGGL((wos_fold4_kernel<3>), dim3(g4), blk, 0, s, prm, tk, n, p, g, nest, steps, nullptr, nullptr);
    } else {
      hipLaunchKernelGGL((wos_fold4_kernel<2>), dim3(g4), blk, 0, s, prm, tk, n, p, g, nest, steps, nullptr, nullptr);
    }
    return hipGetLastError();
  }
  if (p_var || g_var) return hipErrorInvalidValue;
  const int grid = (int)((n + kFoldPoints - 1) / kFoldPoints);
  if (grid < 1) return hipSuccess;
  if (dim == 2)
    hipLaunchKernelGGL(wos_fold_kernel<2>, dim3(grid), dim3(kFoldPoints), 0, s, prm, tk, n, p, g, nest, steps);
  else
    hipLaunchKernelGGL(wos_fold_kernel<3>, dim3(grid), dim3(kFoldPoints), 0, s, prm, tk, n, p, g, nest, steps);
  return hipGetLastError();
}

size_t first_ball_wave_lds_bytes(int lhs_floats, int n_pairs) {
  const int P = fb_points_per_wave(n_pairs);
  return (size_t)2 * P * lhs_floats * sizeof(float) + fb_union_bytes(P * lhs_floats, 2 * n_pairs);
}

int first_ball_points_per_wave(int n_pairs) { return fb_points_per_wave(n_pairs); }

size_t walk_wave_lds_bytes(int dim) { return dim == 2 ? walk_scratch_bytes<2>() : walk_scratch_bytes<3>(); }

hipError_t occupancy_blocks_per_cu(const KernelVariant& v, int which, size_t shmem, int* blocks) {
  const UnitKernels k = kernels_of(v);
  const void* kernel = which == 0 ? (const void*)k.first_ball : which == 1 ? (const void*)k.walk : nullptr;
  if (!kernel) return hipErrorInvalidValue;
  return hipOccupancyMaxActiveBlocksPerMultiprocessor(blocks, kernel, kBlock, shmem);
}
// ... 78 lines not shown
```

### neural-monte-carlo-fluid-simulation_amd/csrc/wos_launch.h

```cpp
#pragma once
#include <hip/hip_runtime.h>
#include "wos_scene.h"
#include "wos_variant.h"

namespace wos {
constexpr int kBlockThreads = 256;
constexpr int kWavesPerBlockHost = 4;
constexpr int kNumCounters = 9;
constexpr int kTaskQueueSlot0 = kNumCounters + 8;
constexpr int kNumCounterSlots = kTaskQueueSlot0 + kMaxTaskQueues * 8;
constexpr int kMainCounterSlots = kNumCounterSlots;

hipError_t launch_first_balls(const KernelVariant& v, const DevScene& sc, const DevParams& prm, const float* pts,
                              int64_t n, int64_t base, int64_t stride, const DevTasks& tk,
                              unsigned long long* counters, unsigned int* work, int grid, size_t shmem, int lhs_floats,
                              hipStream_t s);
hipError_t launch_point_setup(int dim, const DevScene& sc, const DevParams& prm, const float* pts, int64_t n,
                              const DevTasks& tk, hipStream_t s);
hipError_t launch_point_query(int dim, const DevScene& sc, int which, float mask, const float* pts, int64_t n,
                              float* dist, float* sdist, float* closest, int32_t* state, hipStream_t s);
hipError_t launch_zero(unsigned long long* a, int n64, uint32_t* b, int n32, hipStream_t s);
hipError_t launch_lpt_order(const DevTasks& tk, int64_t n, hipStream_t s);
hipError_t launch_walks(const KernelVariant& v, const DevScene& sc, const DevParams& prm, const DevTasks& tk,
                        int64_t base, int64_t stride, unsigned long long* counters, unsigned int* tqueue, int grid,
                        size_t shmem, int geom_floats, hipStream_t s);
hipError_t launch_fold(int dim, const DevParams& prm, const DevTasks& tk, int64_t n, float* p, float* g,
                       int32_t* nest, int32_t* steps, float* p_var, float* g_var, hipStream_t s);
size_t first_ball_wave_lds_bytes(int lhs_floats, int n_pairs);
int first_ball_points_per_wave(int n_pairs);
size_t walk_wave_lds_bytes(int dim);
hipError_t occupancy_blocks_per_cu(const KernelVariant& v, int which, size_t shmem, int* blocks);
void diag_dump(const char* tag);
void diag_dump_bstart(const char* tag);
void diag_print(const char* tag, const void* sym);
hipError_t launch_math_selftest(int which, const double* x, double* out, int64_t n, hipStream_t s);

hipError_t launch_lhs_selftest(int dim, const DevParams& prm, const long long* gidx, int n, float* out, hipStream_t s);
size_t lhs_selftest_lds_bytes(int n_pairs, int dim, int jump_n);
hipError_t launch_lhs_permute_selftest(int impl, const int* partner, const float* values, int nstrat, int sd, int slots,
                                       int count, float* out, hipStream_t s);
int lhs_permute_selftest_slots(int impl);
int lhs_permute_selftest_max_strata(int impl);
void lhs_plan(int n_pairs, int dim, int32_t* out);

hipError_t launch_bvc_point_info(const DevScene& sc, const float* pts, int64_t n, float* dd, float* nd,
                                 int32_t* inside, float* src, hipStream_t s);
hipError_t launch_bvc_start(const DevScene& sc, const DevParams& prm, const float* bpt, const float* bnrm,
                            const uint8_t* aligned, const float* bdd, int64_t nb, const DevTasks& tk, int on_neumann,
                            uint32_t tag, hipStream_t s);
hipError_t launch_bvc_fd(const DevScene& sc, const float* pts, const float* sol, int64_t n, float* dn, hipStream_t s);
hipError_t launch_bvc_fold(const DevTasks& tk, int64_t nb, float* sol, int32_t* nest, hipStream_t s);
hipError_t launch_bvc_splat_list(const float* edd, const float* end_, const int32_t* ein, int64_t ne, float cutoff,
                                 float mask, int double_sided, uint32_t* list, uint32_t* count, hipStream_t s);
hipError_t launch_bvc_splat(const float* recs, int r0, int r1, int first, int last, float* state,
                            const uint32_t* list, const uint32_t* count, const float* ept, int64_t ne,
                            float absorption, float radius_clamp, float reg, float* sol, float* grad, hipStream_t s);
hipError_t launch_bvc_fill(float* recs, int64_t b0, int64_t b1, const float* bsol, const float* bdn,
                           const DevScene& sc, int ignore_neumann, hipStream_t s);
hipError_t launch_first_balls_rec(int dim, const DevScene& sc, const DevParams& prm, const float* pts, int64_t n,
                                  int64_t base, int64_t stride, const DevTasks& tk, const DevTape& tape,
                                  unsigned long long* counters, unsigned int* work, int grid, size_t shmem,
                                  int lhs_floats, hipStream_t s);
hipError_t launch_walks_rec(int dim, bool geom_global, const DevScene& sc, const DevParams& prm, const DevTasks& tk,
                            const DevTape& tape, int64_t base, int64_t stride, unsigned long long* counters,
                            unsigned int* tqueue, int grid, size_t shmem, int geom_floats, hipStream_t s);
hipError_t occupancy_rec_blocks_per_cu(int dim, bool geom_global, int which, size_t shmem, int* blocks);
constexpr int64_t tape_slot_blocks(int64_t T) { return (T + 1 + 2047) / 2048; }
hipError_t launch_tape_slots(const uint32_t* code, int64_t T, uint32_t* slot, unsigned long long* bsum, hipStream_t s);
hipError_t launch_tape_stats(const uint32_t* code, const uint32_t* cnt, int64_t T, unsigned long long* out,
                             hipStream_t s);
hipError_t launch_tape_replay(const DevTape& tape, const uint32_t* code, const DevScene& sc, int ignore_source,
                              int64_t T, float* total, float* first, hipStream_t s);
hipError_t launch_tape_adjoint_fold(int dim, const DevParams& prm, const uint32_t* code, const float* bdir,
                                    const float* sdir, const int32_t* pstate, int64_t n, int64_t T, int wpp,
                                    int n_channels, const float* up_p, const float* up_g, int64_t up_stride,
                                    float* a, float* c, hipStream_t s);
hipError_t launch_tape_scatter(const DevTape& tape, const uint32_t* code, int64_t cells, int n_channels, int64_t T,
                               const float* a, const float* c, float* out, hipStream_t s);
constexpr int kTapeIndexTile = 1024;
struct DevTapeIndex {
  const uint32_t* row;
  const uint32_t* cell;
  const uint32_t* id;
  const float* w;
  float* part;
  uint32_t n_terms;
};
constexpr int64_t tape_index_tiles(int64_t n_terms) { return (n_terms + kTapeIndexTile - 1) / kTapeIndexTile; }
hipError_t launch_tape_index_enum(const DevTape& tape, const uint32_t* code, int64_t T, int64_t slots, int64_t cells,
                                  uint32_t* key, unsigned long long* val, hipStream_t s);
hipError_t tape_index_sort(void* temp, size_t* temp_bytes, const uint32_t* key_in, uint32_t* key_out,
                           const unsigned long long* val_in, unsigned long long* val_out, int64_t N, int bits,
                           hipStream_t s);
hipError_t launch_tape_index_count(const uint32_t* key, int64_t N, uint32_t* n_terms, hipStream_t s);
hipError_t launch_tape_index_finish(const uint32_t* key, const unsigned long long* val, uint32_t n_terms,
                                    int64_t cells, uint32_t* row, uint32_t* cell, uint32_t* id, float* w,
                                    hipStream_t s);
hipError_t launch_tape_rowsum(const DevTapeIndex& ix, int64_t cells, int n_channels, int64_t T, const float* a,
                              const float* c, float* out, hipStream_t s);
hipError_t launch_source_pack(const float* planar, float* texels, int64_t cells, int channels, hipStream_t s);
}
```

### neural-monte-carlo-fluid-simulation_amd/csrc/wos_select.h

```cpp
#pragma once
#include "wos_device.h"
#include "wos_variant.h"

namespace wos {

#define WOS_FIRST_BALL_PARAMS \
  const DevScene, const DevParams, const float*, int64_t, int64_t, int64_t, const DevTasks, unsigned long long*, \
      unsigned int*, int
#define WOS_WALK_PARAMS \
  const DevScene, const DevParams, const DevTasks, int64_t, int64_t, unsigned long long*, unsigned int*, int
using FirstBallKernel = void (*)(WOS_FIRST_BALL_PARAMS);
using WalkKernel = void (*)(WOS_WALK_PARAMS);

struct UnitKernels {
  FirstBallKernel first_ball = nullptr;
  WalkKernel walk = nullptr;
};
UnitKernels unit_kernels_plain(const KernelVariant& v);
UnitKernels unit_kernels_channels(const KernelVariant& v);
UnitKernels unit_kernels_robust(const KernelVariant& v);
UnitKernels unit_kernels_channels_rb(const KernelVariant& v);
UnitKernels unit_kernels_bstart(const KernelVariant& v);

#define WOS_FIRST_BALL_INSTANTIATE(D, R, C) \
  template __global__ void wos_first_ball_kernel<D, R, C>(WOS_FIRST_BALL_PARAMS);
#define WOS_FIRST_BALL_SELECT(D, R, C) \
  if (v.valid && !v.bstart && v.dim == D && v.robust == R && v.channels == C) k.first_ball = wos_first_ball_kernel<D, R, C>;

#define WOS_WALK_INSTANTIATE(D, G, B, R, N, S, C) \
  template __global__ void wos_walk_kernel<D, G, B, R, N, S, C>(WOS_WALK_PARAMS);
#define WOS_WALK_SELECT(D, G, B, R, N, S, C)                                                                  \
  if (v.valid && v.dim == D && v.geom_global == G && v.bstart == B && v.robust == R && v.neumann == N && \
      v.spread == S && v.channels == C)                                                                       \
    k.walk = wos_walk_kernel<D, G, B, R, N, S, C>;

}
```

### neural-monte-carlo-fluid-simulation_amd/csrc/wos_selftest.hip

```cpp
#include "wos_device.h"
#include "wos_launch.h"
#include "../../include/wos.h"

namespace wos {

template <int DIM>
__global__ __launch_bounds__(kWave) void wos_lhs_selftest_kernel(const DevParams prm, const long long* __restrict__ gidx,
                                                                 int n, int lhs_floats, float* __restrict__ out) {
  extern __shared__ __attribute__((aligned(16))) float probe_smem[];
  const int lane = threadIdx.x & (kWave - 1);
  const int npairs = prm.n_pairs, nstrat = 2 * npairs, nd = nstrat * (DIM - 1);
  const int P = fb_points_per_wave(npairs);
  const int wave_floats = 2 * P * lhs_floats + (int)(fb_union_bytes(P * lhs_floats, nstrat) / sizeof(float));
  float* wbase = probe_smem;
  unsigned long long* ljump = reinterpret_cast<unsigned long long*>(probe_smem + wave_floats);
  for (int i = threadIdx.x; i < 2 * prm.lhs_jump_n; i += blockDim.x) ljump[i] = prm.jump[i];
  __syncthreads();
  char* scratch = reinterpret_cast<char*>(wbase + 2 * P * lhs_floats);
  const int first = (int)blockIdx.x * P;
  const int cnt = n - first < P ? n - first : P;
  const bool all = lhs_all_fits(npairs, DIM, P);
  for (int s = 0; s < cnt; s++) {
    float* strat_s = wbase + 2 * s * lhs_floats;
    build_lhs<DIM>(prm, ljump, (int64_t)gidx[first + s], strat_s, reinterpret_cast<int*>(strat_s + lhs_floats), scratch,
                   lane, !all);
  }
  if constexpr (DIM == 3)
    if (all) {
      const int* part0 = reinterpret_cast<const int*>(wbase + lhs_floats);
      if (nstrat <= kWave) lhs_permute_reg<DIM - 1, 1, 4>(wbase, part0, 2 * lhs_floats, 0, cnt * (DIM - 1), nstrat, lane);
      else lhs_permute_reg<DIM - 1, 2, 2>(wbase, part0, 2 * lhs_floats, 0, cnt * (DIM - 1), nstrat, lane);
    }
  wave_sync();
  for (int s = 0; s < cnt; s++) {
    const float* strat_s = wbase + 2 * s * lhs_floats;
    for (int k = lane; k < nd; k += kWave) out[(int64_t)(first + s) * nd + k] = strat_s[k];
  }
}

__global__ __launch_bounds__(kWave) void wos_lhs_permute_selftest_kernel(int impl, const int* __restrict__ partner,
                                                                         const float* __restrict__ values, int nstrat,
                                                                         int sd, int slots, int cap,
                                                                         float* __restrict__ out) {
  extern __shared__ __attribute__((aligned(16))) float probe_smem[];
  const int lane = threadIdx.x & (kWave - 1);
  const int nd = nstrat * sd, lhs_floats = (nd + 3) & ~3;
  float* wbase = probe_smem;
  char* scratch = reinterpret_cast<char*>(wbase + 2 * cap * lhs_floats);
  const int64_t t0 = (int64_t)blockIdx.x * cap * nd;
  for (int s = 0; s < cap; s++) {
    float* strat_s = wbase + 2 * s * lhs_floats;
    int* part_s = reinterpret_cast<int*>(strat_s + lhs_floats);
    for (int k = lane; k < nd; k += kWave) {
      strat_s[k] = values[t0 + (int64_t)s * nd + k];
      part_s[k] = partner[t0 + (int64_t)s * nd + k];
    }
  }
  wave_sync();
  const int* part0 = reinterpret_cast<const int*>(wbase + lhs_floats);
  switch (impl) {
    case WOS_LHS_REG1:
      for (int i = 0; i < sd; ++i) {
        if (sd == 1) lhs_permute_reg<1, 1, 1>(wbase, part0, 0, i, 1, nstrat, lane);
        else lhs_permute_reg<2, 1, 1>(wbase, part0, 0, i, 1, nstrat, lane);
      }
      break;
    case WOS_LHS_REG2:
      for (int i = 0; i < sd; ++i) {
        if (sd == 1) lhs_permute_reg<1, 2, 1>(wbase, part0, 0, i, 1, nstrat, lane);
        else lhs_permute_reg<2, 2, 1>(wbase, part0, 0, i, 1, nstrat, lane);
      }
      break;
    case WOS_LHS_LDS:
      for (int i = 0; i < sd; ++i) lhs_permute(wbase, part0, nstrat, sd, i, scratch, lane);
      break;
    case WOS_LHS_PACK_R1:
      lhs_permute_reg<2, 1, 4>(wbase, part0, 2 * lhs_floats, 0, slots * 2, nstrat, lane);
      break;
    case WOS_LHS_PACK_R2:
      lhs_permute_reg<2, 2, 2>(wbase, part0, 2 * lhs_floats, 0, slots * 2, nstrat, lane);
      break;
    default:
      break;
  }
  wave_sync();
  for (int s = 0; s < cap; s++) {
    const float* strat_s = wbase + 2 * s * lhs_floats;
    for (int k = lane; k < nd; k += kWave) out[t0 + (int64_t)s * nd + k] = strat_s[k];
  }
}

size_t lhs_selftest_lds_bytes(int n_pairs, int dim, int jump_n) {
  const int lhs_floats = ((2 * n_pairs * (dim - 1)) + 3) & ~3;
  const int P = fb_points_per_wave(n_pairs);
  return (size_t)2 * P * lhs_floats * sizeof(float) + fb_union_bytes(P * lhs_floats, 2 * n_pairs) +
         (size_t)jump_n * 2 * sizeof(unsigned long long);
}

hipError_t launch_lhs_selftest(int dim, const DevParams& prm, const long long* gidx, int n, float* out, hipStream_t s) {
  const int lhs_floats = ((2 * prm.n_pairs * (dim - 1)) + 3) & ~3;
  const int P = fb_points_per_wave(prm.n_pairs);
  const int grid = (n + P - 1) / P;
  const size_t shmem = lhs_selftest_lds_bytes(prm.n_pairs, dim, prm.lhs_jump_n);
  if (dim == 2)
    hipLaunchKernelGGL(wos_lhs_selftest_kernel<2>, dim3(grid), dim3(kWave), shmem, s, prm, gidx, n, lhs_floats, out);
  else
    hipLaunchKernelGGL(wos_lhs_selftest_kernel<3>, dim3(grid), dim3(kWave), shmem, s, prm, gidx, n, lhs_floats, out);
  return hipGetLastError();
}

int lhs_permute_selftest_slots(int impl) { return impl == WOS_LHS_PACK_R1 ? 2 : 1; }

int lhs_permute_selftest_max_strata(int impl) {
  switch (impl) {
    case WOS_LHS_REG1: case WOS_LHS_PACK_R1: return kWave;
    case WOS_LHS_REG2: case WOS_LHS_PACK_R2: return 2 * kWave;
    case WOS_LHS_LDS: return 4 * kWave;
    default: return 0;
  }
}

hipError_t launch_lhs_permute_selftest(int impl, const int* partner, const float* values, int nstrat, int sd, int slots,
                                       int count, float* out, hipStream_t s) {
  const int cap = lhs_permute_selftest_slots(impl);
  const int lhs_floats = (nstrat * sd + 3) & ~3;
  const size_t shmem = (size_t)2 * cap * lhs_floats * sizeof(float) + (size_t)28 * lhs_floats + 64;
  hipLaunchKernelGGL(wos_lhs_permute_selftest_kernel, dim3(count), dim3(kWave), shmem, s, impl, partner, values, nstrat,
                     sd, slots, cap, out);
  return hipGetLastError();
}

void lhs_plan(int n_pairs, int dim, int32_t* out) {
  const int nstrat = 2 * n_pairs, P = fb_points_per_wave(n_pairs);
  const int lhs_floats = ((nstrat * (dim - 1)) + 3) & ~3;
  const int draws = 2 * nstrat * (dim - 1);
  out[0] = P;
  out[1] = lhs_all_fits(n_pairs, dim, P) ? 1 : 0;
  out[2] = nstrat <= kWave ? WOS_LHS_REG1 : (nstrat <= 2 * kWave ? WOS_LHS_REG2 : (nstrat <= 4 * kWave ? WOS_LHS_LDS : WOS_LHS_SERIAL));
  out[3] = P > 1 ? 1 : (n_pairs + kWave - 1) / kWave;
  out[4] = draws <= kLhsJumpMax ? 0 : 1;
  out[5] = (int32_t)((size_t)2 * P * lhs_floats * sizeof(float) + fb_union_bytes(P * lhs_floats, nstrat));
  out[6] = 0;
  out[7] = (int32_t)kPtGrab;
  out[8] = nstrat <= 4 * kWave ? (nstrat + kWave - 1) / kWave : 0;
}

}
```

### neural-monte-carlo-fluid-simulation_amd/csrc/wos_tape.hip

```cpp
#include "wos_device.h"
#include "wos_launch.h"
#include "wos_select.h"

namespace wos {

template <int DIM>
__global__ __launch_bounds__(kBlock) __attribute__((amdgpu_waves_per_eu(DIM == 2 ? WOS_FB_WAVES_PER_EU2 : WOS_FB_WAVES_PER_EU))) void wos_first_ball_rec_kernel(
    const DevScene sc, const DevParams prm, const float* __restrict__ pts, int64_t n, int64_t base, int64_t stride,
    const DevTasks tk, unsigned long long* __restrict__ counters, unsigned int* __restrict__ work, int lhs_floats,
    const DevTape tape_arg) {
  constexpr bool RB = false, REC = true;
  constexpr int NC = 1;
  const DevTape* const tape = &tape_arg;
#include "wos_first_ball_body.inc"
}

template <int DIM, bool GG>
__global__ __launch_bounds__(kBlock) __attribute__((amdgpu_waves_per_eu(DIM == 2 ? WOS_WALK_WAVES_PER_EU : WOS_WALK_WAVES_PER_EU3))) void wos_walk_rec_kernel(
    const DevScene sc_arg, const DevParams prm_arg, const DevTasks tk_arg, int64_t base, int64_t stride,
    unsigned long long* __restrict__ counters, unsigned int* __restrict__ tqueue, int geom_floats,
    const DevTape tape_arg) {
  constexpr bool BSTART = false, RB = false, NEU = true, SPR = false, REC = true;
  constexpr int NC = 1;
  const DevTape* const tape = &tape_arg;
#include "wos_walk_body.inc"
}

template __global__ void wos_first_ball_rec_kernel<2>(WOS_FIRST_BALL_PARAMS, const DevTape);
template __global__ void wos_first_ball_rec_kernel<3>(WOS_FIRST_BALL_PARAMS, const DevTape);
template __global__ void wos_walk_rec_kernel<2, false>(WOS_WALK_PARAMS, const DevTape);
template __global__ void wos_walk_rec_kernel<2, true>(WOS_WALK_PARAMS, const DevTape);
template __global__ void wos_walk_rec_kernel<3, false>(WOS_WALK_PARAMS, const DevTape);
template __global__ void wos_walk_rec_kernel<3, true>(WOS_WALK_PARAMS, const DevTape);

using FirstBallRecKernel = void (*)(WOS_FIRST_BALL_PARAMS, const DevTape);
using WalkRecKernel = void (*)(WOS_WALK_PARAMS, const DevTape);

static FirstBallRecKernel first_ball_rec_of(int dim) {
  return dim == 2 ? wos_first_ball_rec_kernel<2> : dim == 3 ? wos_first_ball_rec_kernel<3> : nullptr;
}
static WalkRecKernel walk_rec_of(int dim, bool gg) {
  if (dim == 2) return gg ? wos_walk_rec_kernel<2, true> : wos_walk_rec_kernel<2, false>;
  if (dim == 3) return gg ? wos_walk_rec_kernel<3, true> : wos_walk_rec_kernel<3, false>;
  return nullptr;
}

hipError_t launch_first_balls_rec(int dim, const DevScene& sc, const DevParams& prm, const float* pts, int64_t n,
                                  int64_t base, int64_t stride, const DevTasks& tk, const DevTape& tape,
                                  unsigned long long* counters, unsigned int* work, int grid, size_t shmem,
                                  int lhs_floats, hipStream_t s) {
  const FirstBallRecKernel kernel = first_ball_rec_of(dim);
  if (!kernel) return hipErrorInvalidValue;
  hipLaunchKernelGGL(kernel, dim3(grid), dim3(kBlock), shmem, s, sc, prm, pts, n, base, stride, tk, counters, work,
                     lhs_floats, tape);
  return hipGetLastError();
}

hipError_t launch_walks_rec(int dim, bool geom_global, const DevScene& sc, const DevParams& prm, const DevTasks& tk,
                            const DevTape& tape, int64_t base, int64_t stride, unsigned long long* counters,
                            unsigned int* tqueue, int grid, size_t shmem, int geom_floats, hipStream_t s) {
  const WalkRecKernel kernel = walk_rec_of(dim, geom_global);
  if (!kernel) return hipErrorInvalidValue;
  hipLaunchKernelGGL(kernel, dim3(grid), dim3(kBlock), shmem, s, sc, prm, tk, base, stride, counters, tqueue,
                     geom_floats, tape);
  return hipGetLastError();
}

hipError_t occupancy_rec_blocks_per_cu(int dim, bool geom_global, int which, size_t shmem, int* blocks) {
  const void* kernel = which == 0 ? (const void*)first_ball_rec_of(dim)
                                  : which == 1 ? (const void*)walk_rec_of(dim, geom_global) : nullptr;
  if (!kernel) return hipErrorInvalidValue;
  return hipOccupancyMaxActiveBlocksPerMultiprocessor(blocks, kernel, kBlock, shmem);
}

constexpr int kSlotPer = 8, kSlotBlock = 256 * kSlotPer;

__device__ __forceinline__ uint32_t tape_cap_of(uint32_t code) { return (code & 1u) && (code >> 1) > 0u ? (code >> 1) - 1u : 0u; }

__device__ __forceinline__ unsigned long long block_excl_scan_256(unsigned long long v, unsigned long long* sh,
                                                                  unsigned long long* sum) {
  const int tid = threadIdx.x;
  sh[tid] = v;
  __syncthreads();
  for (int off = 1; off < 256; off <<= 1) {
    const unsigned long long a = tid >= off ? sh[tid - off] : 0ull;
    __syncthreads();
    sh[tid] += a;
    __syncthreads();
  }
  const unsigned long long incl = sh[tid];
  *sum = sh[255];
  __syncthreads();
  return incl - v;
}

__global__ __launch_bounds__(256) void wos_tape_cap_sum_kernel(const uint32_t* __restrict__ code, int64_t T,
                                                               unsigned long long* __restrict__ bsum) {
  __shared__ unsigned long long sh[256];
  const int64_t b0 = (int64_t)blockIdx.x * kSlotBlock;
  unsigned long long v = 0ull;
  for (int j = 0; j < kSlotPer; j++) {
    const int64_t i = b0 + (int64_t)j * 256 + threadIdx.x;
    if (i < T) v += tape_cap_of(code[i]);
  }
  unsigned long long sum;
  block_excl_scan_256(v, sh, &sum);
  if (threadIdx.x == 0) bsum[blockIdx.x] = sum;
}

__global__ __launch_bounds__(256) void wos_tape_block_scan_kernel(unsigned long long* bsum, int64_t nb) {
  __shared__ unsigned long long sh[256];
  unsigned long long carry = 0ull;
  for (int64_t b0 = 0; b0 < nb; b0 += 256) {
    const int64_t i = b0 + threadIdx.x;
    const unsigned long long v = i < nb ? bsum[i] : 0ull;
    unsigned long long sum;
    const unsigned long long ex = block_excl_scan_256(v, sh, &sum);
    if (i < nb) bsum[i] = carry + ex;
    carry += sum;
  }
  if (threadIdx.x == 0) bsum[nb] = carry;
}

__global__ __launch_bounds__(256) void wos_tape_slot_kernel(const uint32_t* __restrict__ code, int64_t T,
                                                            const unsigned long long* __restrict__ bsum,
                                                            uint32_t* __restrict__ slot) {
  __shared__ unsigned long long sh[256];
  const int64_t i0 = (int64_t)blockIdx.x * kSlotBlock + (int64_t)threadIdx.x * kSlotPer;
  uint32_t cap[kSlotPer];
  unsigned long long v = 0ull;
  for (int j = 0; j < kSlotPer; j++) {
    cap[j] = i0 + j < T ? tape_cap_of(code[i0 + j]) : 0u;
    v += cap[j];
  }
  unsigned long long sum;
  unsigned long long at = bsum[blockIdx.x] + block_excl_scan_256(v, sh, &sum);
  for (int j = 0; j < kSlotPer; j++) {
// ... 375 lines not shown
```

### neural-monte-carlo-fluid-simulation_amd/wos_amd/__init__.py

```python
from ._lib import WosError, load as load_library
from . import siren
from .engine import WalkTape, WosScene, bvc_params, load_obj, solver_params, selftest_math, selftest_lhs, selftest_lhs_permute, selftest_lhs_permute_slots, selftest_lhs_plan, selftest_tape_rowsum, device_count, release_caches, set_max_batch_tasks

__all__ = ["WalkTape", "WosScene", "WosError", "bvc_params", "load_obj", "solver_params", "selftest_math", "selftest_lhs", "selftest_lhs_permute",
           "selftest_lhs_permute_slots", "selftest_lhs_plan", "selftest_tape_rowsum", "device_count", "set_max_batch_tasks",
           "load_library", "release_caches", "siren"]
```

### neural-monte-carlo-fluid-simulation_amd/wos_amd/_lib.py

```python
import ctypes as C
import os

PKG_DIR = os.path.dirname(os.path.dirname(os.path.abspath(__file__)))
LIB_PATH = os.environ.get("WOS_LIB_PATH") or os.path.join(PKG_DIR, "lib", "libwos_hip.so")

ABI_VERSION = 10
WOS_OK = 0
WOS_E_CAPACITY = -4
WOS_PTRS_DEVICE = 0x1
WOS_ASYNC = 0x2
MAX_CHANNELS = 4
LHS_REG1, LHS_REG2, LHS_LDS, LHS_PACK_R1, LHS_PACK_R2, LHS_SERIAL = range(6)


class WosError(RuntimeError):
    pass


class Mesh(C.Structure):
    _fields_ = [("dim", C.c_int32), ("n_vertices", C.c_int32), ("n_prims", C.c_int32),
                ("vertices", C.POINTER(C.c_float)), ("prims", C.POINTER(C.c_int32))]


class SceneDesc(C.Structure):
# ... 12 lines not shown
        ("neumann_image_box", C.c_float * 4), ("neumann_image_on_device", C.c_int32),
    ]


class SceneInfo(C.Structure):
    _fields_ = [("dim", C.c_int32), ("n_prims", C.c_int32), ("n_silhouettes", C.c_int32),
                ("n_dprims", C.c_int32), ("device", C.c_int32),
                ("bbox_min", C.c_float * 3), ("bbox_max", C.c_float * 3)]


class SolverParams(C.Structure):
    _fields_ = [
        ("n_walks", C.c_int32), ("max_walk_length", C.c_int32),
        ("steps_before_tikhonov", C.c_int32), ("steps_before_maximal_spheres", C.c_int32),
        ("epsilon_shell", C.c_float), ("min_star_radius", C.c_float),
        ("silhouette_precision", C.c_float), ("russian_roulette_threshold", C.c_float),
        ("boundary_distance_mask", C.c_float),
        ("disable_gradient_control_variates", C.c_int32),
        ("disable_gradient_antithetic_variates", C.c_int32),
        ("use_cosine_sampling", C.c_int32), ("ignore_dirichlet", C.c_int32),
        ("ignore_neumann", C.c_int32), ("ignore_source", C.c_int32),
        ("seed", C.c_uint64),
        ("robust_float", C.c_int32),
        ("schedule", C.c_uint32),
    ]


SCHED_GEOM_GLOBAL = 0x1
SCHED_FULL_NEUMANN = 0x2
SCHED_NO_STAR_GRID = 0x4
SCHED_NO_DIR_GRID = 0x8
SCHED_NO_TAIL_SPREAD = 0x10
SCHED_NO_GRID_SPREAD = 0x20


class BvcParams(C.Structure):
    _fields_ = [("n_walks_solution", C.c_int32), ("n_walks_gradient", C.c_int32),
                ("boundary_cache_size", C.c_int32), ("domain_cache_size", C.c_int32),
                ("grid_res", C.c_int32), ("use_finite_differences", C.c_int32),
                ("normal_offset", C.c_float), ("radius_clamp", C.c_float),
                ("kernel_regularization", C.c_float), ("grid_box", C.c_float * 4)]


class Stats(C.Structure):
    _fields_ = [(n, C.c_uint64) for n in (
        "walk_steps", "wasted_steps", "walks_recorded", "walks_escaped", "walks_max_length",
        "walks_rr", "walks_dirichlet", "points_estimated", "rejection_iters")] + [
        (n, C.c_double) for n in ("kernel_ms", "first_ball_ms", "walk_ms", "fold_ms")] + [("walk_launches", C.c_uint64)] + [
        (n, C.c_int32) for n in ("first_ball_blocks_per_cu", "walk_blocks_per_cu", "walk_lds_bytes", "star_grid",
                                 "geom_global", "dir_grid")] + [("ticket", C.c_uint64)]

    def as_dict(self):
        return {n: (float(getattr(self, n)) if t is C.c_double else int(getattr(self, n))) for n, t in self._fields_}


class TapeInfo(C.Structure):
    _fields_ = [("dim", C.c_int32), ("n_walks", C.c_int32), ("source_dims", C.c_int32 * 3), ("device", C.c_int32),
                ("n_points", C.c_int64), ("n_tasks", C.c_int64), ("n_entries", C.c_int64),
                ("max_entries_per_walk", C.c_int64), ("bytes", C.c_int64), ("replay_chunk_entries", C.c_int32)]


class TapeIndexInfo(C.Structure):
    _fields_ = [("built", C.c_int32), ("n_segments", C.c_int32), ("n_terms", C.c_int64), ("n_cells", C.c_int64),
                ("max_terms_per_cell", C.c_int64), ("bytes", C.c_int64), ("tile_terms", C.c_int32)]


class SirenNet(C.Structure):
    _fields_ = [("d_in", C.c_int32), ("d_out", C.c_int32), ("hidden", C.c_int32), ("n_hidden_layers", C.c_int32),
                ("omega", C.c_float), ("weights", C.POINTER(C.c_void_p)), ("biases", C.POINTER(C.c_void_p))]


EXPORTS = (
    "wos_load_obj", "wos_mesh_free", "wos_scene_create", "wos_scene_destroy",
    "wos_scene_get_info", "wos_scene_set_source", "wos_release_caches", "wos_default_params", "wos_solve", "wos_solve_var",
    "wos_solve_stats", "wos_default_bvc_params", "wos_bvc",
    "wos_selftest_math", "wos_selftest_lhs", "wos_selftest_lhs_permute", "wos_selftest_lhs_plan", "wos_last_error", "wos_abi_version", "wos_device_count", "wos_set_max_batch_tasks",
    "wos_scene_set_source_channels", "wos_scene_channels", "wos_solve_channels",
    "wos_tape_record", "wos_tape_solve", "wos_tape_get_info", "wos_tape_destroy",
    "wos_tape_vjp", "wos_tape_read",
    "wos_tape_index_build", "wos_tape_index_get_info", "wos_tape_index_read", "wos_tape_vjp_indexed",
    "wos_selftest_tape_rowsum",
    "wos_scene_query",
    "wos_siren_eval", "wos_selftest_siren_layer",
)

QUERY_NEUMANN, QUERY_DIRICHLET = 0, 1
STATE_ESTIMATED, STATE_MASK_P, STATE_MASK_GRAD, STATE_INSIDE = 1, 2, 4, 8

TAPE_FIELDS = {"code": (0, "u4"), "cnt": (1, "u4"), "slot": (2, "u4"), "cell0": (3, "u4"), "gnorm": (4, "f4"),
               "thr_end": (5, "f4"), "term": (6, "f4"), "tneu": (7, "f4"), "bdir": (8, "f4"), "sdir": (9, "f4"),
               "cell": (10, "u4"), "thr": (11, "f4"), "nrm": (12, "f4"), "pstate": (13, "i4")}
TAPE_SEGMENT_POINTS = 14
TAPE_INDEX_FIELDS = {"row": (0, "u4"), "id": (1, "u4"), "w": (2, "f4"), "cell": (3, "u4")}

_lib = None


def load():
    global _lib
    if _lib is not None:
        return _lib
    if not os.path.exists(LIB_PATH):
        raise WosError(f"{LIB_PATH} not built: run `make -C {PKG_DIR}` or __graft_entry__.build()")
    L = C.CDLL(LIB_PATH)
    L.wos_load_obj.restype = C.c_int
    L.wos_load_obj.argtypes = [C.c_char_p, C.c_int32, C.c_int32, C.c_int32, C.POINTER(Mesh)]
    L.wos_mesh_free.restype = None
    L.wos_mesh_free.argtypes = [C.POINTER(Mesh)]
    L.wos_scene_create.restype = C.c_int
    L.wos_scene_create.argtypes = [C.POINTER(SceneDesc), C.c_int32, C.POINTER(C.c_void_p)]
    L.wos_scene_destroy.restype = C.c_int
    L.wos_scene_destroy.argtypes = [C.c_void_p]
    L.wos_scene_get_info.restype = C.c_int
    L.wos_scene_get_info.argtypes = [C.c_void_p, C.POINTER(SceneInfo)]
    L.wos_scene_set_source.restype = C.c_int
    L.wos_scene_set_source.argtypes = [C.c_void_p, C.c_void_p, C.POINTER(C.c_int32), C.c_int32, C.c_void_p]
    L.wos_scene_query.restype = C.c_int
    L.wos_scene_query.argtypes = [C.c_void_p, C.c_int32, C.c_float, C.c_void_p, C.c_int64, C.c_void_p, C.c_void_p,
                                  C.c_void_p, C.c_void_p, C.c_void_p, C.c_uint32]
    L.wos_release_caches.restype = C.c_int
    L.wos_release_caches.argtypes = [C.c_int32]
    L.wos_set_max_batch_tasks.restype = C.c_int64
    L.wos_set_max_batch_tasks.argtypes = [C.c_int64]
    L.wos_default_params.restype = None
    L.wos_default_params.argtypes = [C.POINTER(SolverParams)]
    L.wos_solve.restype = C.c_int
    L.wos_solve.argtypes = [C.c_void_p, C.POINTER(SolverParams), C.c_void_p, C.c_int64, C.c_int64,
                            C.c_int64, C.c_void_p, C.c_void_p, C.c_void_p, C.c_void_p,
                            C.POINTER(Stats), C.c_void_p, C.c_uint32]
    L.wos_solve_var.restype = C.c_int
    L.wos_solve_var.argtypes = [C.c_void_p, C.POINTER(SolverParams), C.c_void_p, C.c_int64, C.c_int64,
                                C.c_int64, C.c_void_p, C.c_void_p, C.c_void_p, C.c_void_p, C.c_void_p,
                                C.c_void_p, C.POINTER(Stats), C.c_void_p, C.c_uint32]
    L.wos_scene_set_source_channels.restype = C.c_int
    L.wos_scene_set_source_channels.argtypes = [C.c_void_p, C.c_void_p, C.c_int32, C.POINTER(C.c_int32),
                                                C.POINTER(C.c_float), C.c_int32, C.c_void_p]
    L.wos_scene_channels.restype = C.c_int32
    L.wos_scene_channels.argtypes = [C.c_void_p]
    L.wos_solve_channels.restype = C.c_int
    L.wos_solve_channels.argtypes = [C.c_void_p, C.POINTER(SolverParams), C.c_void_p, C.c_int64, C.c_int64,
                                     C.c_int64, C.c_int32, C.c_void_p, C.c_void_p, C.c_void_p, C.c_void_p,
                                     C.c_void_p, C.c_void_p, C.POINTER(Stats), C.c_void_p, C.c_uint32]
    L.wos_solve_stats.restype = C.c_int
    L.wos_solve_stats.argtypes = [C.c_void_p, C.c_uint64, C.POINTER(Stats)]
    L.wos_tape_record.restype = C.c_int
    L.wos_tape_record.argtypes = [C.c_void_p, C.POINTER(SolverParams), C.c_void_p, C.c_int64, C.c_int64, C.c_int64,
                                  C.c_int64, C.POINTER(C.c_void_p), C.POINTER(Stats), C.c_void_p, C.c_uint32]
    L.wos_tape_solve.restype = C.c_int
    L.wos_tape_solve.argtypes = [C.c_void_p, C.c_void_p, C.c_int32, C.c_void_p, C.c_void_p, C.c_void_p, C.c_void_p,
                                 C.c_void_p, C.c_void_p, C.POINTER(Stats), C.c_void_p, C.c_uint32]
    L.wos_tape_get_info.restype = C.c_int
    L.wos_tape_get_info.argtypes = [C.c_void_p, C.POINTER(TapeInfo)]
    L.wos_tape_destroy.restype = C.c_int
    L.wos_tape_destroy.argtypes = [C.c_void_p]
    L.wos_tape_vjp.restype = C.c_int
    L.wos_tape_vjp.argtypes = [C.c_void_p, C.c_void_p, C.c_int32, C.c_void_p, C.c_void_p, C.c_void_p,
                               C.POINTER(Stats), C.c_void_p, C.c_uint32]
    L.wos_tape_read.restype = C.c_int
    L.wos_tape_read.argtypes = [C.c_void_p, C.c_int32, C.c_int32, C.c_int64, C.c_int64, C.c_void_p]
    L.wos_tape_index_build.restype = C.c_int
    L.wos_tape_index_build.argtypes = [C.c_void_p, C.c_int64]
    L.wos_tape_index_get_info.restype = C.c_int
    L.wos_tape_index_get_info.argtypes = [C.c_void_p, C.POINTER(TapeIndexInfo)]
    L.wos_tape_index_read.restype = C.c_int
    L.wos_tape_index_read.argtypes = [C.c_void_p, C.c_int32, C.c_int32, C.c_int64, C.c_int64, C.c_void_p]
    L.wos_tape_vjp_indexed.restype = C.c_int
    L.wos_tape_vjp_indexed.argtypes = L.wos_tape_vjp.argtypes
    L.wos_selftest_tape_rowsum.restype = C.c_int
    L.wos_selftest_tape_rowsum.argtypes = [C.c_void_p, C.c_int64, C.c_void_p, C.c_void_p, C.c_void_p, C.c_void_p,
                                           C.c_int64, C.c_int32, C.c_void_p, C.POINTER(C.c_int32), C.c_int32]
    L.wos_siren_eval.restype = C.c_int
    L.wos_siren_eval.argtypes = [C.POINTER(SirenNet), C.c_void_p, C.c_int64, C.c_void_p, C.c_void_p, C.c_void_p,
                                 C.c_uint32, C.c_int32, C.c_void_p]
    L.wos_selftest_siren_layer.restype = C.c_int
    L.wos_selftest_siren_layer.argtypes = [C.c_int32, C.c_int32, C.c_int64, C.c_void_p, C.c_void_p, C.c_void_p,
                                           C.c_void_p, C.c_int32]
    L.wos_default_bvc_params.restype = None
    L.wos_default_bvc_params.argtypes = [C.POINTER(BvcParams)]
    L.wos_bvc.restype = C.c_int
    L.wos_bvc.argtypes = [C.c_void_p, C.POINTER(SolverParams), C.POINTER(BvcParams), C.c_void_p, C.c_void_p,
                          C.c_void_p, C.c_int64, C.c_void_p, C.POINTER(Stats)]
    L.wos_selftest_math.restype = C.c_int
    L.wos_selftest_math.argtypes = [C.c_int32, C.c_void_p, C.c_void_p, C.c_int64, C.c_int32]
    L.wos_selftest_lhs.restype = C.c_int
    L.wos_selftest_lhs.argtypes = [C.c_uint64, C.c_void_p, C.c_int64, C.c_int32, C.c_int32, C.c_int32, C.c_void_p,
                                   C.c_int32]
    L.wos_selftest_lhs_permute.restype = C.c_int
    L.wos_selftest_lhs_permute.argtypes = [C.c_int32, C.c_void_p, C.c_void_p, C.c_int32, C.c_int32, C.c_int32,
                                           C.c_int32, C.c_void_p, C.c_int32]
    L.wos_selftest_lhs_plan.restype = C.c_int
    L.wos_selftest_lhs_plan.argtypes = [C.c_int32, C.c_int32, C.c_void_p]
    L.wos_last_error.restype = C.c_char_p
    L.wos_last_error.argtypes = []
    L.wos_abi_version.restype = C.c_int32
    L.wos_device_count.restype = C.c_int32
    if L.wos_abi_version() != ABI_VERSION:
        raise WosError(f"{LIB_PATH}: ABI {L.wos_abi_version()} != binding ABI {ABI_VERSION}; rebuild the library")
    _lib = L
    return L


def check(rc, what=""):
    if rc != WOS_OK:
        msg = load().wos_last_error().decode(errors="replace")
        raise WosError(f"{what} failed ({rc}): {msg}")
```

### neural-monte-carlo-fluid-simulation_amd/wos_amd/engine.py

```python
import ctypes as C
import os

import numpy as np

from . import _lib
from ._lib import BvcParams, SceneDesc, SceneInfo, SolverParams, Stats, WosError, check

_DEFAULT_SEED = 0x5EED0001


def load_obj(path, dim, flip_orientation=False, normalize=False):
    L = _lib.load()
    m = _lib.Mesh()
    check(L.wos_load_obj(os.fsencode(path), dim, int(flip_orientation), int(normalize), C.byref(m)),
          f"wos_load_obj({path})")
    try:
        v = np.ctypeslib.as_array(m.vertices, shape=(m.n_vertices * dim,)).copy().reshape(-1, dim)
        ix = np.ctypeslib.as_array(m.prims, shape=(m.n_prims * dim,)).copy().reshape(-1, dim)
    finally:
        L.wos_mesh_free(C.byref(m))
    return v.astype(np.float32), ix.astype(np.int32)


def _get_opt(d, key, default, typ):
# ... 519 lines not shown
                raise WosError(f"WalkTape.vjp: {name} must have shape {shp}, got {tuple(u.shape)}")
        if sc.source_shape is None:
            raise WosError("WalkTape.vjp: the scene has no source grid")
        on_dev = any(_is_torch(u) and u.is_cuda for u in (grad_p, grad_grad))
        st = Stats()
        if on_dev:
            import torch
            dev = next(u.device for u in (grad_p, grad_grad) if _is_torch(u) and u.is_cuda)
            up = [None if u is None else torch.as_tensor(u).detach().to(dev, torch.float32).contiguous()
                  for u in (grad_p, grad_grad)]
            out = torch.empty(sc.source_shape, dtype=torch.float32, device=dev)
            cur = torch.cuda.current_stream(dev)
            if stream is None:
                s = cur.cuda_stream
            else:
                ts = stream if isinstance(stream, torch.cuda.Stream) else torch.cuda.ExternalStream(int(stream),
                                                                                                    device=dev)
                s = ts.cuda_stream
                ts.wait_stream(cur)
            ptr = lambda t: t.data_ptr() if t is not None else None
            flags = _lib.WOS_PTRS_DEVICE
        else:
            up = [None if u is None else np.ascontiguousarray(u.detach().cpu().numpy() if _is_torch(u) else u,
                                                              dtype=np.float32) for u in (grad_p, grad_grad)]
            out = np.empty(sc.source_shape, np.float32)
            ptr = lambda a: a.ctypes.data if a is not None else None
            s, flags = stream, 0
        if deterministic:
            self.build_index()
        fn = "wos_tape_vjp_indexed" if deterministic else "wos_tape_vjp"
        check(getattr(L, fn)(self._h, sc._h, nch, ptr(up[0]), ptr(up[1]), ptr(out), C.byref(st), s, flags), fn)
        self.last_vjp_stats = st.as_dict()
        return out

    def read(self, field, segment=0):
        L = _lib.load()
        if field not in _lib.TAPE_FIELDS:
            raise WosError(f"WalkTape.read: unknown field {field!r} (one of {', '.join(_lib.TAPE_FIELDS)})")
        fid, dtype = _lib.TAPE_FIELDS[field]
        npts = np.zeros(1, np.int64)
        check(L.wos_tape_read(self._h, segment, _lib.TAPE_SEGMENT_POINTS, 0, 1, npts.ctypes.data), "wos_tape_read")
        info = self.info
        T = int(npts[0]) * (info["n_tasks"] // max(1, info["n_points"]))
        dim = info["dim"]
        if field in ("cell", "thr", "nrm"):
            last = np.zeros(1, np.uint32)
            check(L.wos_tape_read(self._h, segment, _lib.TAPE_FIELDS["slot"][0], T, 1, last.ctypes.data), "wos_tape_read")
            shape = (int(last[0]),)
        else:
            shape = {"slot": (T + 1,), "bdir": (dim, T), "sdir": (dim, T), "pstate": (int(npts[0]),)}.get(field, (T,))
        out = np.empty(shape, dtype)
        check(L.wos_tape_read(self._h, segment, fid, 0, out.size, out.ctypes.data), "wos_tape_read")
        return out

    @property
    def segments(self):
        L = _lib.load()
        out, npts = [], np.zeros(1, np.int64)
        while sum(out) < self._n:
            check(L.wos_tape_read(self._h, len(out), _lib.TAPE_SEGMENT_POINTS, 0, 1, npts.ctypes.data), "wos_tape_read")
            out.append(int(npts[0]))
        return out

    def close(self):
        if getattr(self, "_h", None):
            _lib.load().wos_tape_destroy(self._h)
            self._h = None

    def __del__(self):
        try:
            self.close()
        except Exception:
            pass


def release_caches(device=-1):
    check(_lib.load().wos_release_caches(int(device)), "wos_release_caches")


def set_max_batch_tasks(n):
    return int(_lib.load().wos_set_max_batch_tasks(int(n)))


def selftest_math(which, x, device=0):
    x = np.ascontiguousarray(x, dtype=np.float64)
    out = np.empty_like(x)
    check(_lib.load().wos_selftest_math(which, x.ctypes.data, out.ctypes.data, x.size, device),
          "wos_selftest_math")
    return out


def selftest_lhs(key, gidx, n_pairs, dim, jump_lds=True, device=0):
    gidx = np.ascontiguousarray(gidx, dtype=np.int64).reshape(-1)
    out = np.empty((gidx.size, 2 * int(n_pairs), int(dim) - 1), np.float32)
    check(_lib.load().wos_selftest_lhs(int(key), gidx.ctypes.data, gidx.size, int(n_pairs), int(dim),
                                       int(bool(jump_lds)), out.ctypes.data, device), "wos_selftest_lhs")
    return out


def selftest_lhs_permute_slots(impl):
    return 2 if impl == _lib.LHS_PACK_R1 else 1


def selftest_lhs_permute(impl, partner, values, slots=1, device=0):
    partner = np.ascontiguousarray(partner, dtype=np.int32)
    values = np.ascontiguousarray(values, dtype=np.float32)
    cap = selftest_lhs_permute_slots(impl)
    if partner.ndim != 4 or values.ndim != 4 or partner.shape[1] != cap or \
            values.shape != (partner.shape[0], cap, partner.shape[3], partner.shape[2]):
        raise WosError(f"partner must be [count, {cap}, sd, nstrat] and values [count, {cap}, nstrat, sd]")
    count, _, sd, nstrat = partner.shape
    out = np.empty_like(values)
    check(_lib.load().wos_selftest_lhs_permute(int(impl), partner.ctypes.data, values.ctypes.data, nstrat, sd,
                                               int(slots), count, out.ctypes.data, device),
          "wos_selftest_lhs_permute")
    return out


def selftest_lhs_plan(n_pairs, dim):
    out = np.zeros(9, np.int32)
    check(_lib.load().wos_selftest_lhs_plan(int(n_pairs), int(dim), out.ctypes.data), "wos_selftest_lhs_plan")
    keys = ("points_per_wave", "one_pass", "shuffle", "pair_passes", "jump_mixed", "wave_lds_bytes", "lds_budget",
            "point_grab", "shuffle_chunks")
    return {k: int(v) for k, v in zip(keys, out)}


def selftest_tape_rowsum(row, id, w, a, c, device=0):
    row = np.ascontiguousarray(row, dtype=np.uint32)
    id = np.ascontiguousarray(id, dtype=np.uint32)
    w = np.ascontiguousarray(w, dtype=np.float32)
    a = np.ascontiguousarray(a, dtype=np.float32)
    c = np.ascontiguousarray(c, dtype=np.float32)
    if a.shape != c.shape or a.ndim not in (1, 2) or id.shape != w.shape or row.ndim != 1 or row.size < 2:
        raise WosError("selftest_tape_rowsum: row [n_rows + 1], id / w [n_terms], a / c [C, T] or [T]")
    nch = 1 if a.ndim == 1 else a.shape[0]
    if id.size != int(row[-1]):
        raise WosError(f"selftest_tape_rowsum: {id.size} terms, row[-1] = {int(row[-1])}")
    out = np.empty((nch, row.size - 1), np.float32)
    tile = C.c_int32(0)
    check(_lib.load().wos_selftest_tape_rowsum(row.ctypes.data, row.size - 1, id.ctypes.data, w.ctypes.data,
                                               a.ctypes.data, c.ctypes.data, a.shape[-1], nch, out.ctypes.data,
                                               C.byref(tile), device), "wos_selftest_tape_rowsum")
    return (out[0] if a.ndim == 1 else out), int(tile.value)


def device_count():
    return int(_lib.load().wos_device_count())
```

Measured before the change: 6.214 billion.

## Cache per-point stratified LHS samples in a device table reused across solves

```diff
diff --git a/include/wos.h b/include/wos.h
--- a/include/wos.h
+++ b/include/wos.h
@@ -76,6 +76,10 @@
 
 int64_t wos_set_max_batch_tasks(int64_t max_tasks);
 
+int64_t wos_set_lhs_table_bytes(int64_t bytes);
+int wos_lhs_table_info(int32_t device, int64_t out[8]);
+int wos_lhs_table_read(int32_t device, int64_t row0, int64_t nrows, float *out);
+
 typedef struct wos_scene_info {
     int32_t dim, n_prims, n_silhouettes, n_dprims, device;
     float bbox_min[3], bbox_max[3];
diff --git a/neural-monte-carlo-fluid-simulation_amd/csrc/wos_capi.hip b/neural-monte-carlo-fluid-simulation_amd/csrc/wos_capi.hip
--- a/neural-monte-carlo-fluid-simulation_amd/csrc/wos_capi.hip
+++ b/neural-monte-carlo-fluid-simulation_amd/csrc/wos_capi.hip
@@ -17,6 +17,7 @@
 #include "wos_detmath.h"
 #include "wos_host_scene.h"
 #include "wos_launch.h"
+#include "wos_lhs_table.h"
 #include "wos_siren.h"
 
 namespace {
@@ -100,6 +101,8 @@
   TaskWs side[kSideWs];
   hipStream_t bvc_dir = nullptr;
   hipEvent_t bvc_dir_done = nullptr;
+  float* d_lhs = nullptr;
+  wos::LhsTableState lhs;
 };
 
 constexpr int kMaxDevices = 64;
@@ -112,6 +115,9 @@
   c.ws_var_points = 0;
   hipFree(c.d_jump); hipFree(c.d_tasks); hipFree(c.d_pstate); hipFree(c.d_counters); hipFree(c.d_rejtab);
   c.d_rejtab = nullptr;
+  hipFree(c.d_lhs);
+  c.d_lhs = nullptr;
+  c.lhs = wos::LhsTableState{};
   for (StatSlot& q : c.slot) {
     if (q.ev0) hipEventDestroy(q.ev0);
     if (q.ev1) hipEventDestroy(q.ev1);
@@ -314,6 +320,12 @@
 static_assert(WOS_BATCH_LOG2 <= 30, "task indices carry a flag in bit 31 (wos_walk_kernel hand-out)");
 constexpr int64_t kDefaultBatchTasks = (int64_t)1 << WOS_BATCH_LOG2;
 std::atomic<int64_t> g_max_batch_tasks{kDefaultBatchTasks};
+int64_t lhs_table_bytes_default() {
+  const char* e = std::getenv("WOS_LHS_TABLE_BYTES");
+  if (!e || !*e) return wos::kLhsTableDefaultBytes;
+  return std::max<int64_t>(0, std::strtoll(e, nullptr, 10));
+}
+std::atomic<int64_t> g_lhs_table_bytes{lhs_table_bytes_default()};
 std::atomic<uint64_t> g_scene_serial{0};
 
 }
@@ -642,6 +654,43 @@
   const int64_t v = max_tasks <= 0 ? kDefaultBatchTasks
                                    : std::min<int64_t>(std::max<int64_t>(max_tasks, (int64_t)1 << 16), (int64_t)1 << 30);
   return g_max_batch_tasks.exchange(v);
+}
+
+int64_t wos_set_lhs_table_bytes(int64_t bytes) { return g_lhs_table_bytes.exchange(std::max<int64_t>(bytes, 0)); }
+
+int wos_lhs_table_info(int32_t device, int64_t out[8]) {
+  int ndev = 0;
+  if (!out || device < 0 || device >= kMaxDevices || hipGetDeviceCount(&ndev) != hipSuccess || device >= ndev)
+    return fail(WOS_E_INVALID, "wos_lhs_table_info: bad argument");
+  DevCtx& c = g_ctx[device];
+  std::lock_guard<std::mutex> lk(c.mu);
+  const int64_t rf = c.lhs.rows > 0 ? wos::lhs_row_floats(c.lhs.key) : 0;
+  out[0] = c.lhs.rows;
+  out[1] = rf;
+  out[2] = c.lhs.rows * rf * (int64_t)sizeof(float);
+  out[3] = c.lhs.builds;
+  out[4] = c.lhs.hits;
+  out[5] = c.lhs.inline_solves;
+  out[6] = (int64_t)c.lhs.key.seed;
+  out[7] = g_lhs_table_bytes.load();
+  return WOS_OK;
+}
+
+int wos_lhs_table_read(int32_t device, int64_t row0, int64_t nrows, float* out) {
+  int ndev = 0;
+  if (!out || device < 0 || device >= kMaxDevices || hipGetDeviceCount(&ndev) != hipSuccess || device >= ndev)
+    return fail(WOS_E_INVALID, "wos_lhs_table_read: bad argument");
+  DevCtx& c = g_ctx[device];
+  std::lock_guard<std::mutex> lk(c.mu);
+  if (row0 < 0 || nrows < 0 || row0 > c.lhs.rows || nrows > c.lhs.rows - row0)
+    return fail(WOS_E_INVALID, "wos_lhs_table_read: rows " + std::to_string(row0) + " .. " + std::to_string(row0 + nrows) +
+                                   " of a table of " + std::to_string(c.lhs.rows));
+  if (nrows == 0) return WOS_OK;
+  HIP_TRY(hipSetDevice(device));
+  if (c.inflight) HIP_TRY(hipEventSynchronize(c.done));
+  const int64_t rf = wos::lhs_row_floats(c.lhs.key);
+  HIP_TRY(hipMemcpy(out, c.d_lhs + row0 * rf, (size_t)(nrows * rf) * sizeof(float), hipMemcpyDeviceToHost));
+  return WOS_OK;
 }
 
 int wos_release_caches(int32_t device) {
@@ -1001,6 +1050,7 @@
   float* p_var = nullptr;
   float* grad_var = nullptr;
   int channels = 1;
+  bool no_lhs_table = false;
 };
 
 int solve_locked(wos_scene* s, const wos_solver_params* prm, const float* pts, int64_t n, int64_t index_base,
@@ -1189,6 +1239,48 @@
   return WOS_OK;
 }
 
+int lhs_table_for_solve(DevCtx& c, int dim, const wos::DevParams& dp, int64_t n, int64_t index_base, int64_t index_stride,
+                        hipStream_t st, const float** tab) {
+  *tab = nullptr;
+  wos::LhsKey key;
+  key.seed = dp.seed;
+  key.index_base = index_base;
+  key.index_stride = index_stride;
+  key.n_pairs = dp.n_pairs;
+  key.n_anti = dp.n_anti;
+  key.dim = dim;
+  const wos::LhsDecision d = wos::lhs_table_decide(c.lhs, key, n, g_lhs_table_bytes.load());
+  if (d.drop) {
+    hipFree(c.d_lhs);
+    c.d_lhs = nullptr;
+  }
+  if (d.action == wos::kLhsHit) {
+    *tab = c.d_lhs;
+    return WOS_OK;
+  }
+  if (d.action != wos::kLhsBuild) return WOS_OK;
+  wos::DevParams fp = dp;
+  fp.lhs_jump_n = std::min(2 * (2 * dp.n_pairs) * (dim - 1), wos::kLhsJumpMax);
+  if (wos::lhs_selftest_lds_bytes(dp.n_pairs, dim, fp.lhs_jump_n) > 64 * 1024) fp.lhs_jump_n = 0;
+  const size_t bytes = (size_t)(d.rows * wos::lhs_row_floats(key)) * sizeof(float);
+  if (wos::lhs_selftest_lds_bytes(dp.n_pairs, dim, 0) > 64 * 1024 ||
+      hipMalloc((void**)&c.d_lhs, bytes) != hipSuccess) {
+    (void)hipGetLastError();
+    c.d_lhs = nullptr;
+    wos::lhs_table_failed(c.lhs);
+    return WOS_OK;
+  }
+  if (wos::launch_lhs_fill(dim, fp, index_base, index_stride, d.rows, c.d_lhs, st) != hipSuccess) {
+    hipFree(c.d_lhs);
+    c.d_lhs = nullptr;
+    wos::lhs_table_failed(c.lhs);
+    return fail(WOS_E_DEVICE, "wos_solve: the stratified-sample table's fill did not launch");
+  }
+  wos::lhs_table_built(c.lhs, d.rows);
+  *tab = c.d_lhs;
+  return WOS_OK;
+}
+
 int solve_locked(wos_scene* s, const wos_solver_params* prm, const float* pts, int64_t n, int64_t index_base,
                  int64_t index_stride, float* p, float* grad, int32_t* n_est, int32_t* steps, wos_stats* stats,
                  void* stream, uint32_t flags, const SolveExtra& ex) {
@@ -1251,6 +1343,12 @@
   }
   const int grid_fb = plan.grid_fb, grid_walk = plan.grid_walk, bpc_fb = plan.bpc_fb, bpc_walk = plan.bpc_walk;
   const size_t shmem_fb_run = plan.shmem_fb_run;
+  const float* lhs_tab = nullptr;
+  if (!ex.no_lhs_table) {
+    int rc = lhs_table_for_solve(c, dim, dp, n, index_base, index_stride, st, &lhs_tab);
+    if (rc != WOS_OK) return rc;
+  }
+  const int64_t lhs_row = (int64_t)2 * dp.n_pairs * (dim - 1);
   const uint64_t ticket = c.next_ticket++;
   StatSlot& q = c.slot[ticket % kStatSlots];
   while ((int64_t)q.bev.size() < 4 * n_chunks) {
@@ -1287,7 +1385,8 @@
     HIP_TRY(wos::launch_point_setup(dim, dfb, dp, d_pts + b0 * dim, nb, tk, st));
     HIP_TRY(wos::launch_lpt_order(tk, nb, st));
     HIP_TRY(wos::launch_first_balls(kv, dfb, dp, d_pts + b0 * dim, nb, bbase, index_stride, tk, c.d_counters,
-                                    q_points, grid_fb, shmem_fb_run, lhs_floats, st));
+                                    q_points, grid_fb, shmem_fb_run, lhs_floats,
+                                    lhs_tab ? lhs_tab + b0 * lhs_row : nullptr, st));
     HIP_TRY(hipEventRecord(ev[1], st));
     HIP_TRY(wos::launch_walks(kv, dsc, dp, tk, bbase, index_stride, c.d_counters, q_tasks, walk_grid,
                               shmem_walk, geom_floats_walk, st));
@@ -2342,6 +2441,7 @@
     SolveExtra ex;
     ex.force_estimate = true;
     ex.wave_prio = 2;
+    ex.no_lhs_table = true;
     for (const Run& r : runs) {
       if (!r.dir) continue;
       ex.ddir = d_ddir + 2 * r.b0;
diff --git a/neural-monte-carlo-fluid-simulation_amd/csrc/wos_device.h b/neural-monte-carlo-fluid-simulation_amd/csrc/wos_device.h
--- a/neural-monte-carlo-fluid-simulation_amd/csrc/wos_device.h
+++ b/neural-monte-carlo-fluid-simulation_amd/csrc/wos_device.h
@@ -3214,10 +3214,14 @@
   if (threadIdx.x < kCostBuckets && s_hist[threadIdx.x]) atomicAdd(&tk.hist[threadIdx.x], s_hist[threadIdx.x]);
 }
 
+#ifndef WOS_LHS_TAB_PREFETCH
+#define WOS_LHS_TAB_PREFETCH 1
+#endif
 template <int DIM, bool RB = false, int NC = 1>
 __global__ __launch_bounds__(kBlock) __attribute__((amdgpu_waves_per_eu(DIM == 2 ? WOS_FB_WAVES_PER_EU2 : WOS_FB_WAVES_PER_EU))) void wos_first_ball_kernel(
     const DevScene sc, const DevParams prm, const float* __restrict__ pts, int64_t n, int64_t base, int64_t stride,
-    const DevTasks tk, unsigned long long* __restrict__ counters, unsigned int* __restrict__ work, int lhs_floats) {
+    const DevTasks tk, unsigned long long* __restrict__ counters, unsigned int* __restrict__ work, int lhs_floats,
+    const float* __restrict__ lhs_tab) {
   constexpr bool REC = false;
   const DevTape* const tape = nullptr;
 #include "wos_first_ball_body.inc"
diff --git a/neural-monte-carlo-fluid-simulation_amd/csrc/wos_first_ball_body.inc b/neural-monte-carlo-fluid-simulation_amd/csrc/wos_first_ball_body.inc
--- a/neural-monte-carlo-fluid-simulation_amd/csrc/wos_first_ball_body.inc
+++ b/neural-monte-carlo-fluid-simulation_amd/csrc/wos_first_ball_body.inc
@@ -31,6 +31,11 @@
   bool en = false;
   const bool pre = !RB && DIM == 2 && yuk0;
   float bn[4] = {0.0f, 0.0f, 0.0f, 0.0f};
+  constexpr int SD = DIM - 1;
+  using LhsTuple = typename std::conditional<DIM == 2, float2, float4>::type;
+  const bool tabm = lhs_tab != nullptr;
+  const bool tload = tabm && used && wl < npairs;
+  LhsTuple tn{};
   {
     const unsigned int li = idx + (unsigned int)myslot;
     for (int k = 0; k < DIM; k++) xn[k] = (int64_t)li < n ? pts[(int64_t)li * DIM + k] : 0.0f;
@@ -39,6 +44,8 @@
       en = (tk.pstate[li] & kPtEstimate) != 0;
       if (pre)
         for (int k = 0; k < 4; k++) bn[k] = tk.pball[k * tk.pball_stride + li];
+      if (WOS_LHS_TAB_PREFETCH && tload)
+        tn = *reinterpret_cast<const LhsTuple*>(lhs_tab + (int64_t)li * (2 * npairs * SD) + 2 * SD * wl);
     }
   }
   for (;;) {
@@ -49,6 +56,7 @@
     const bool estimate = en && used;
     float pb[4];
     for (int k = 0; k < 4; k++) pb[k] = bn[k];
+    const LhsTuple tc = tn;
     const bool grab = idx + (unsigned int)P >= cend;
     unsigned int nidx_l0 = 0;
     if (grab && lane == 0) nidx_l0 = atomicAdd(work, take);
@@ -69,6 +77,8 @@
         en = (tk.pstate[li] & kPtEstimate) != 0;
         if (pre)
           for (int k = 0; k < 4; k++) bn[k] = tk.pball[k * tk.pball_stride + li];
+        if (WOS_LHS_TAB_PREFETCH && tload)
+        tn = *reinterpret_cast<const LhsTuple*>(lhs_tab + (int64_t)li * (2 * npairs * SD) + 2 * SD * wl);
       }
     }
     const uint64_t em = __ballot(estimate && wl == 0);
@@ -77,20 +87,36 @@
     DIAG_ADD(D_FB_SETUP, t_fb0);
     DIAG_COUNT(D_FB_PTS, __popcll(em));
     DIAG_T0(t_fb1);
-    const bool all = lhs_all_fits(npairs, DIM, P);
-    for (int s = 0; s < P; s++) {
-      if (!all && !((em >> (s * span)) & 1ull)) continue;
-      float* strat_s = wbase + 2 * s * lhs_floats;
-      build_lhs<DIM>(prm, ljump, base + (int64_t)(idx + (unsigned int)s) * stride, strat_s,
-                     reinterpret_cast<int*>(strat_s + lhs_floats), reinterpret_cast<char*>(rejL), lane, !all);
+    if (tabm) {
+#if WOS_LHS_TAB_PREFETCH
+      if (tload) *reinterpret_cast<LhsTuple*>(wbase + 2 * myslot * lhs_floats + 2 * SD * wl) = tc;
+#else
+      (void)tc;
+      if (tload && (int64_t)(idx + (unsigned int)myslot) < n)
+        *reinterpret_cast<LhsTuple*>(wbase + 2 * myslot * lhs_floats + 2 * SD * wl) = *reinterpret_cast<const LhsTuple*>(
+            lhs_tab + (int64_t)(idx + (unsigned int)myslot) * (2 * npairs * SD) + 2 * SD * wl);
+#endif
+      if (P == 1)
+        for (int w = kWave + lane; w < npairs; w += kWave)
+          *reinterpret_cast<LhsTuple*>(wbase + 2 * SD * w) =
+              *reinterpret_cast<const LhsTuple*>(lhs_tab + (int64_t)idx * (2 * npairs * SD) + 2 * SD * w);
+      wave_sync();
+    } else {
+      const bool all = lhs_all_fits(npairs, DIM, P);
+      for (int s = 0; s < P; s++) {
+        if (!all && !((em >> (s * span)) & 1ull)) continue;
+        float* strat_s = wbase + 2 * s * lhs_floats;
+        build_lhs<DIM>(prm, ljump, base + (int64_t)(idx + (unsigned int)s) * stride, strat_s,
+                       reinterpret_cast<int*>(strat_s + lhs_floats), reinterpret_cast<char*>(rejL), lane, !all);
+      }
+      if constexpr (DIM == 3)
+        if (all) {
+          const int ns = 2 * npairs;
+          const int* part0 = reinterpret_cast<const int*>(wbase + lhs_floats);
+          if (ns <= kWave) lhs_permute_reg<DIM - 1, 1, 4>(wbase, part0, 2 * lhs_floats, 0, P * (DIM - 1), ns, lane);
+          else lhs_permute_reg<DIM - 1, 2, 2>(wbase, part0, 2 * lhs_floats, 0, P * (DIM - 1), ns, lane);
+        }
     }
-    if constexpr (DIM == 3)
-      if (all) {
-        const int ns = 2 * npairs;
-        const int* part0 = reinterpret_cast<const int*>(wbase + lhs_floats);
-        if (ns <= kWave) lhs_permute_reg<DIM - 1, 1, 4>(wbase, part0, 2 * lhs_floats, 0, P * (DIM - 1), ns, lane);
-        else lhs_permute_reg<DIM - 1, 2, 2>(wbase, part0, 2 * lhs_floats, 0, P * (DIM - 1), ns, lane);
-      }
     DIAG_ADD(D_FB_LHS, t_fb1);
     DIAG_T0(t_fb2);
     const int fs = (int)(__builtin_ctzll(em) / (unsigned)span);
diff --git a/neural-monte-carlo-fluid-simulation_amd/csrc/wos_kernel.hip b/neural-monte-carlo-fluid-simulation_amd/csrc/wos_kernel.hip
--- a/neural-monte-carlo-fluid-simulation_amd/csrc/wos_kernel.hip
+++ b/neural-monte-carlo-fluid-simulation_amd/csrc/wos_kernel.hip
@@ -116,11 +116,11 @@
 hipError_t launch_first_balls(const KernelVariant& v, const DevScene& sc, const DevParams& prm, const float* pts,
                               int64_t n, int64_t base, int64_t stride, const DevTasks& tk,
                               unsigned long long* counters, unsigned int* work, int grid, size_t shmem, int lhs_floats,
-                              hipStream_t s) {
+                              const float* lhs_tab, hipStream_t s) {
   const FirstBallKernel kernel = kernels_of(v).first_ball;
   if (!kernel) return hipErrorInvalidValue;
   hipLaunchKernelGGL(kernel, dim3(grid), dim3(kBlock), shmem, s, sc, prm, pts, n, base, stride, tk, counters, work,
-                     lhs_floats);
+                     lhs_floats, lhs_tab);
   return hipGetLastError();
 }
 
diff --git a/neural-monte-carlo-fluid-simulation_amd/csrc/wos_launch.h b/neural-monte-carlo-fluid-simulation_amd/csrc/wos_launch.h
--- a/neural-monte-carlo-fluid-simulation_amd/csrc/wos_launch.h
+++ b/neural-monte-carlo-fluid-simulation_amd/csrc/wos_launch.h
@@ -14,7 +14,7 @@
 hipError_t launch_first_balls(const KernelVariant& v, const DevScene& sc, const DevParams& prm, const float* pts,
                               int64_t n, int64_t base, int64_t stride, const DevTasks& tk,
                               unsigned long long* counters, unsigned int* work, int grid, size_t shmem, int lhs_floats,
-                              hipStream_t s);
+                              const float* lhs_tab, hipStream_t s);
 hipError_t launch_point_setup(int dim, const DevScene& sc, const DevParams& prm, const float* pts, int64_t n,
                               const DevTasks& tk, hipStream_t s);
 hipError_t launch_point_query(int dim, const DevScene& sc, int which, float mask, const float* pts, int64_t n,
@@ -37,6 +37,8 @@
 
 hipError_t launch_lhs_selftest(int dim, const DevParams& prm, const long long* gidx, int n, float* out, hipStream_t s);
 size_t lhs_selftest_lds_bytes(int n_pairs, int dim, int jump_n);
+hipError_t launch_lhs_fill(int dim, const DevParams& prm, int64_t base, int64_t stride, int64_t rows, float* out,
+                           hipStream_t s);
 hipError_t launch_lhs_permute_selftest(int impl, const int* partner, const float* values, int nstrat, int sd, int slots,
                                        int count, float* out, hipStream_t s);
 int lhs_permute_selftest_slots(int impl);
diff --git a/neural-monte-carlo-fluid-simulation_amd/csrc/wos_lhs_table.h b/neural-monte-carlo-fluid-simulation_amd/csrc/wos_lhs_table.h
--- /dev/null
+++ b/neural-monte-carlo-fluid-simulation_amd/csrc/wos_lhs_table.h
@@ -0,0 +1,85 @@
+#pragma once
+#include <cstdint>
+
+namespace wos {
+
+struct LhsKey {
+  uint64_t seed = 0;
+  int64_t index_base = 0, index_stride = 0;
+  int32_t n_pairs = 0, n_anti = 0, dim = 0;
+};
+
+inline bool lhs_key_equal(const LhsKey& a, const LhsKey& b) {
+  return a.seed == b.seed && a.index_base == b.index_base && a.index_stride == b.index_stride &&
+         a.n_pairs == b.n_pairs && a.n_anti == b.n_anti && a.dim == b.dim;
+}
+
+inline int64_t lhs_row_floats(const LhsKey& k) { return (int64_t)2 * k.n_pairs * (k.dim - 1); }
+
+constexpr int64_t kLhsTableDefaultBytes = (int64_t)256 << 20;
+
+struct LhsTableState {
+  bool seen = false;
+  LhsKey key;
+  int64_t rows = 0;
+  int64_t builds = 0, hits = 0, inline_solves = 0;
+};
+
+enum LhsAction { kLhsInline = 0, kLhsBuild = 1, kLhsHit = 2 };
+
+struct LhsDecision {
+  LhsAction action = kLhsInline;
+  int64_t rows = 0;
+  bool drop = false;
+};
+
+inline LhsDecision lhs_table_decide(LhsTableState& st, const LhsKey& key, int64_t n, int64_t cap_bytes) {
+  LhsDecision d;
+  const int64_t row_bytes = lhs_row_floats(key) * (int64_t)sizeof(float);
+  if (cap_bytes <= 0 || row_bytes <= 0) {
+    d.drop = st.rows > 0;
+    st.rows = 0;
+    st.seen = false;
+    st.inline_solves++;
+    return d;
+  }
+  if (!st.seen || !lhs_key_equal(st.key, key)) {
+    d.drop = st.rows > 0;
+    st.rows = 0;
+    st.seen = true;
+    st.key = key;
+    st.inline_solves++;
+    return d;
+  }
+  if (n <= 0) return d;
+  if (st.rows >= n) {
+    st.hits++;
+    d.action = kLhsHit;
+    return d;
+  }
+  const int64_t max_rows = cap_bytes / row_bytes;
+  if (n > max_rows) {
+    st.inline_solves++;
+    return d;
+  }
+  const int64_t want = n + n / 8 + 64;
+  d.action = kLhsBuild;
+  d.rows = want <= max_rows ? want : n;
+  d.drop = st.rows > 0;
+  st.rows = 0;
+  return d;
+}
+
+inline void lhs_table_built(LhsTableState& st, int64_t rows) {
+  st.rows = rows;
+  st.builds++;
+  st.hits++;
+}
+
+inline void lhs_table_failed(LhsTableState& st) {
+  st.rows = 0;
+  st.seen = false;
+  st.inline_solves++;
+}
+
+}
diff --git a/neural-monte-carlo-fluid-simulation_amd/csrc/wos_select.h b/neural-monte-carlo-fluid-simulation_amd/csrc/wos_select.h
--- a/neural-monte-carlo-fluid-simulation_amd/csrc/wos_select.h
+++ b/neural-monte-carlo-fluid-simulation_amd/csrc/wos_select.h
@@ -6,7 +6,7 @@
 
 #define WOS_FIRST_BALL_PARAMS \
   const DevScene, const DevParams, const float*, int64_t, int64_t, int64_t, const DevTasks, unsigned long long*, \
-      unsigned int*, int
+      unsigned int*, int, const float*
 #define WOS_WALK_PARAMS \
   const DevScene, const DevParams, const DevTasks, int64_t, int64_t, unsigned long long*, unsigned int*, int
 using FirstBallKernel = void (*)(WOS_FIRST_BALL_PARAMS);
diff --git a/neural-monte-carlo-fluid-simulation_amd/csrc/wos_selftest.hip b/neural-monte-carlo-fluid-simulation_amd/csrc/wos_selftest.hip
--- a/neural-monte-carlo-fluid-simulation_amd/csrc/wos_selftest.hip
+++ b/neural-monte-carlo-fluid-simulation_amd/csrc/wos_selftest.hip
@@ -6,7 +6,8 @@
 
 template <int DIM>
 __global__ __launch_bounds__(kWave) void wos_lhs_selftest_kernel(const DevParams prm, const long long* __restrict__ gidx,
-                                                                 int n, int lhs_floats, float* __restrict__ out) {
+                                                                 int64_t base, int64_t stride, int64_t n, int lhs_floats,
+                                                                 float* __restrict__ out) {
   extern __shared__ __attribute__((aligned(16))) float probe_smem[];
   const int lane = threadIdx.x & (kWave - 1);
   const int npairs = prm.n_pairs, nstrat = 2 * npairs, nd = nstrat * (DIM - 1);
@@ -17,13 +18,13 @@
   for (int i = threadIdx.x; i < 2 * prm.lhs_jump_n; i += blockDim.x) ljump[i] = prm.jump[i];
   __syncthreads();
   char* scratch = reinterpret_cast<char*>(wbase + 2 * P * lhs_floats);
-  const int first = (int)blockIdx.x * P;
-  const int cnt = n - first < P ? n - first : P;
+  const int64_t first = (int64_t)blockIdx.x * P;
+  const int cnt = n - first < P ? (int)(n - first) : P;
   const bool all = lhs_all_fits(npairs, DIM, P);
   for (int s = 0; s < cnt; s++) {
     float* strat_s = wbase + 2 * s * lhs_floats;
-    build_lhs<DIM>(prm, ljump, (int64_t)gidx[first + s], strat_s, reinterpret_cast<int*>(strat_s + lhs_floats), scratch,
-                   lane, !all);
+    const int64_t gi = gidx ? (int64_t)gidx[first + s] : base + (first + s) * stride;
+    build_lhs<DIM>(prm, ljump, gi, strat_s, reinterpret_cast<int*>(strat_s + lhs_floats), scratch, lane, !all);
   }
   if constexpr (DIM == 3)
     if (all) {
@@ -34,7 +35,7 @@
   wave_sync();
   for (int s = 0; s < cnt; s++) {
     const float* strat_s = wbase + 2 * s * lhs_floats;
-    for (int k = lane; k < nd; k += kWave) out[(int64_t)(first + s) * nd + k] = strat_s[k];
+    for (int k = lane; k < nd; k += kWave) out[(first + s) * nd + k] = strat_s[k];
   }
 }
 
@@ -97,16 +98,30 @@
          (size_t)jump_n * 2 * sizeof(unsigned long long);
 }
 
-hipError_t launch_lhs_selftest(int dim, const DevParams& prm, const long long* gidx, int n, float* out, hipStream_t s) {
+static hipError_t launch_lhs_rows(int dim, const DevParams& prm, const long long* gidx, int64_t base, int64_t stride,
+                                  int64_t n, float* out, hipStream_t s) {
   const int lhs_floats = ((2 * prm.n_pairs * (dim - 1)) + 3) & ~3;
   const int P = fb_points_per_wave(prm.n_pairs);
-  const int grid = (n + P - 1) / P;
+  const int64_t grid = (n + P - 1) / P;
+  if (grid < 1) return hipSuccess;
+  if (grid > 0x7FFFFFFFLL) return hipErrorInvalidValue;
   const size_t shmem = lhs_selftest_lds_bytes(prm.n_pairs, dim, prm.lhs_jump_n);
   if (dim == 2)
-    hipLaunchKernelGGL(wos_lhs_selftest_kernel<2>, dim3(grid), dim3(kWave), shmem, s, prm, gidx, n, lhs_floats, out);
+    hipLaunchKernelGGL(wos_lhs_selftest_kernel<2>, dim3((unsigned)grid), dim3(kWave), shmem, s, prm, gidx, base, stride, n,
+                       lhs_floats, out);
   else
-    hipLaunchKernelGGL(wos_lhs_selftest_kernel<3>, dim3(grid), dim3(kWave), shmem, s, prm, gidx, n, lhs_floats, out);
+    hipLaunchKernelGGL(wos_lhs_selftest_kernel<3>, dim3((unsigned)grid), dim3(kWave), shmem, s, prm, gidx, base, stride, n,
+                       lhs_floats, out);
   return hipGetLastError();
+}
+
+hipError_t launch_lhs_selftest(int dim, const DevParams& prm, const long long* gidx, int n, float* out, hipStream_t s) {
+  return launch_lhs_rows(dim, prm, gidx, 0, 0, n, out, s);
+}
+
+hipError_t launch_lhs_fill(int dim, const DevParams& prm, int64_t base, int64_t stride, int64_t rows, float* out,
+                           hipStream_t s) {
+  return launch_lhs_rows(dim, prm, nullptr, base, stride, rows, out, s);
 }
 
 int lhs_permute_selftest_slots(int impl) { return impl == WOS_LHS_PACK_R1 ? 2 : 1; }
diff --git a/neural-monte-carlo-fluid-simulation_amd/csrc/wos_tape.hip b/neural-monte-carlo-fluid-simulation_amd/csrc/wos_tape.hip
--- a/neural-monte-carlo-fluid-simulation_amd/csrc/wos_tape.hip
+++ b/neural-monte-carlo-fluid-simulation_amd/csrc/wos_tape.hip
@@ -8,7 +8,7 @@
 __global__ __launch_bounds__(kBlock) __attribute__((amdgpu_waves_per_eu(DIM == 2 ? WOS_FB_WAVES_PER_EU2 : WOS_FB_WAVES_PER_EU))) void wos_first_ball_rec_kernel(
     const DevScene sc, const DevParams prm, const float* __restrict__ pts, int64_t n, int64_t base, int64_t stride,
     const DevTasks tk, unsigned long long* __restrict__ counters, unsigned int* __restrict__ work, int lhs_floats,
-    const DevTape tape_arg) {
+    const float* __restrict__ lhs_tab, const DevTape tape_arg) {
   constexpr bool RB = false, REC = true;
   constexpr int NC = 1;
   const DevTape* const tape = &tape_arg;
@@ -52,7 +52,7 @@
   const FirstBallRecKernel kernel = first_ball_rec_of(dim);
   if (!kernel) return hipErrorInvalidValue;
   hipLaunchKernelGGL(kernel, dim3(grid), dim3(kBlock), shmem, s, sc, prm, pts, n, base, stride, tk, counters, work,
-                     lhs_floats, tape);
+                     lhs_floats, (const float*)nullptr, tape);
   return hipGetLastError();
 }
 
diff --git a/neural-monte-carlo-fluid-simulation_amd/wos_amd/__init__.py b/neural-monte-carlo-fluid-simulation_amd/wos_amd/__init__.py
--- a/neural-monte-carlo-fluid-simulation_amd/wos_amd/__init__.py
+++ b/neural-monte-carlo-fluid-simulation_amd/wos_amd/__init__.py
@@ -1,7 +1,7 @@
 from ._lib import WosError, load as load_library
 from . import siren
-from .engine import WalkTape, WosScene, bvc_params, load_obj, solver_params, selftest_math, selftest_lhs, selftest_lhs_permute, selftest_lhs_permute_slots, selftest_lhs_plan, selftest_tape_rowsum, device_count, release_caches, set_max_batch_tasks
+from .engine import WalkTape, WosScene, bvc_params, load_obj, solver_params, selftest_math, selftest_lhs, selftest_lhs_permute, selftest_lhs_permute_slots, selftest_lhs_plan, selftest_tape_rowsum, device_count, release_caches, set_max_batch_tasks, set_lhs_table_bytes, lhs_table_info, lhs_table_read
 
 __all__ = ["WalkTape", "WosScene", "WosError", "bvc_params", "load_obj", "solver_params", "selftest_math", "selftest_lhs", "selftest_lhs_permute",
-           "selftest_lhs_permute_slots", "selftest_lhs_plan", "selftest_tape_rowsum", "device_count", "set_max_batch_tasks",
+           "selftest_lhs_permute_slots", "selftest_lhs_plan", "selftest_tape_rowsum", "device_count", "set_max_batch_tasks", "set_lhs_table_bytes", "lhs_table_info", "lhs_table_read",
            "load_library", "release_caches", "siren"]
diff --git a/neural-monte-carlo-fluid-simulation_amd/wos_amd/_lib.py b/neural-monte-carlo-fluid-simulation_amd/wos_amd/_lib.py
--- a/neural-monte-carlo-fluid-simulation_amd/wos_amd/_lib.py
+++ b/neural-monte-carlo-fluid-simulation_amd/wos_amd/_lib.py
@@ -118,6 +118,7 @@
     "wos_selftest_tape_rowsum",
     "wos_scene_query",
     "wos_siren_eval", "wos_selftest_siren_layer",
+    "wos_set_lhs_table_bytes", "wos_lhs_table_info", "wos_lhs_table_read",
 )
 
 QUERY_NEUMANN, QUERY_DIRICHLET = 0, 1
@@ -158,6 +159,12 @@
     L.wos_release_caches.argtypes = [C.c_int32]
     L.wos_set_max_batch_tasks.restype = C.c_int64
     L.wos_set_max_batch_tasks.argtypes = [C.c_int64]
+    L.wos_set_lhs_table_bytes.restype = C.c_int64
+    L.wos_set_lhs_table_bytes.argtypes = [C.c_int64]
+    L.wos_lhs_table_info.restype = C.c_int
+    L.wos_lhs_table_info.argtypes = [C.c_int32, C.POINTER(C.c_int64)]
+    L.wos_lhs_table_read.restype = C.c_int
+    L.wos_lhs_table_read.argtypes = [C.c_int32, C.c_int64, C.c_int64, C.c_void_p]
     L.wos_default_params.restype = None
     L.wos_default_params.argtypes = [C.POINTER(SolverParams)]
     L.wos_solve.restype = C.c_int
diff --git a/neural-monte-carlo-fluid-simulation_amd/wos_amd/engine.py b/neural-monte-carlo-fluid-simulation_amd/wos_amd/engine.py
--- a/neural-monte-carlo-fluid-simulation_amd/wos_amd/engine.py
+++ b/neural-monte-carlo-fluid-simulation_amd/wos_amd/engine.py
@@ -625,6 +625,26 @@
     return int(_lib.load().wos_set_max_batch_tasks(int(n)))
 
 
+def set_lhs_table_bytes(n):
+    return int(_lib.load().wos_set_lhs_table_bytes(int(n)))
+
+
+def lhs_table_info(device=0):
+    out = (C.c_int64 * 8)()
+    check(_lib.load().wos_lhs_table_info(int(device), out), "wos_lhs_table_info")
+    keys = ("rows", "row_floats", "bytes", "builds", "hits", "inline_solves", "seed", "cap_bytes")
+    info = {k: int(v) for k, v in zip(keys, out)}
+    info["seed"] &= (1 << 64) - 1
+    return info
+
+
+def lhs_table_read(row0, nrows, device=0):
+    rf = lhs_table_info(device)["row_floats"]
+    out = np.empty((int(nrows), rf), np.float32)
+    check(_lib.load().wos_lhs_table_read(int(device), int(row0), int(nrows), out.ctypes.data), "wos_lhs_table_read")
+    return out
+
+
 def selftest_math(which, x, device=0):
     x = np.ascontiguousarray(x, dtype=np.float64)
     out = np.empty_like(x)
```

Result: no change. 6.207 billion (-0.1%).
